# gvanhorn38/multibox

Hardware: AMD Instinct MI355X
Metric: images/sec (299x299, 5-AR priors) train (higher is better)
Workload: dtype bf16; 1 GPU; full train step: Inception-ResNet-v2 + multibox heads fwd, on-device matching+loss, bwd, RMSProp+EMA; 299x299, k=5 (P=646), BATCH_SIZE=64/GPU, MAX_NUM_BBOXES=13; global_batch=64, parallelism=dp1, hip_graph=True

## Files before the change

### include/mbx.h

```cpp
#ifndef MBX_H
#define MBX_H

#include <stddef.h>
#include <stdint.h>

#ifdef __cplusplus
extern "C" {
#endif

typedef void* mbx_stream_t;

typedef enum {
  MBX_OK = 0,
  MBX_ERR_INVALID_ARG = -1,
  MBX_ERR_UNSUPPORTED = -2,
  MBX_ERR_LAUNCH = -3,
  MBX_ERR_WORKSPACE = -4
} mbx_status;

int mbx_version(void);
const char* mbx_status_string(int status);

int mbx_priors_count(int k, const int* grids, int n_grids);

// ... 13 lines not shown
              void* workspace, size_t workspace_bytes, mbx_stream_t stream);

int mbx_match_extend(const float* priors , const float* gt ,
                     const int32_t* n_gt , const int32_t* status ,
                     float iou_threshold, int B, int P, int G,
                     int32_t* match ,
                     int32_t* n_extra , mbx_stream_t stream);

int mbx_match_atss_supported(int P, int G, int n_levels, const int32_t* level_start , int topk);
int mbx_match_atss(const float* priors , const int32_t* level_start ,
                   int n_levels, const float* gt , const int32_t* n_gt ,
                   const int32_t* status , int topk, int B, int P, int G,
                   int32_t* match , int32_t* n_extra ,
                   double* thr , mbx_stream_t stream);

size_t mbx_loss_workspace_bytes(int B);
int mbx_loss_fwd_bwd(const float* decoded , const float* conf_in ,
                     int conf_is_logit, const float* gt ,
                     const int32_t* match , float alpha, float grad_scale, int B, int P,
                     int G, float* loss2 ,
                     float* d_raw_locs , float* d_logits ,
                     void* workspace, size_t workspace_bytes, mbx_stream_t stream);

size_t mbx_loss_mined_workspace_bytes(int B, int P);
int mbx_loss_fwd_bwd_mined(const float* decoded , const float* conf_in ,
                           int conf_is_logit, const float* gt ,
                           const int32_t* match , float alpha, float grad_scale, int B, int P,
                           int G, float* loss2 ,
                           float* d_raw_locs , float* d_logits ,
                           int neg_per_pos, int min_neg, int32_t* n_neg ,
                           void* workspace, size_t workspace_bytes, mbx_stream_t stream);

size_t mbx_loss_focal_workspace_bytes(int B, int P);
int mbx_loss_fwd_bwd_focal(const float* decoded , const float* conf_in ,
                           int conf_is_logit, const float* gt ,
                           const int32_t* match , float alpha, float grad_scale, int B, int P,
                           int G, float* loss2 ,
                           float* d_raw_locs , float* d_logits ,
                           float gamma, float w_pos, float w_neg,
                           int neg_per_pos , int min_neg, int32_t* n_neg ,
                           void* workspace, size_t workspace_bytes, mbx_stream_t stream);

enum { MBX_LOC_L2 = 0, MBX_LOC_SMOOTH_L1 = 1, MBX_LOC_GIOU = 2, MBX_LOC_DIOU = 3, MBX_LOC_CIOU = 4 };
size_t mbx_loss_loc_workspace_bytes(int B, int P);
int mbx_loss_fwd_bwd_loc(const float* decoded , const float* conf_in ,
                         int conf_is_logit, const float* gt ,
                         const int32_t* match , float alpha, float grad_scale, int B, int P,
                         int G, float* loss2 ,
                         float* d_raw_locs , float* d_logits ,
                         int loc_type , float loc_beta ,
                         float gamma, float w_pos, float w_neg,
                         int neg_per_pos , int min_neg, int32_t* n_neg ,
                         void* workspace, size_t workspace_bytes, mbx_stream_t stream);

typedef struct {
  int32_t offset_y, offset_x;
  int32_t patch_h, patch_w;
  int32_t image_h, image_w;
  int32_t is_flipped;
  int32_t max_to_keep;
  float restrictions[4];
} mbx_patch_meta;

int mbx_decode_filter_topk(const float* raw_locs , const float* conf ,
                           const float* priors , const mbx_patch_meta* meta ,
                           int B, int P, int k_max, double* out_boxes ,
                           float* out_scores , int32_t* out_index ,
                           int32_t* out_count , mbx_stream_t stream);

int mbx_nms(double* boxes , float* scores , int32_t* index ,
            int32_t* count , int B, int k_max, double iou_threshold, mbx_stream_t stream);

#define MBX_MERGE_MAX_CANDIDATES 16384
int mbx_merge_detections(const double* boxes , const float* scores ,
                         const int32_t* count , const int32_t* image_rows , int I, int k_max,
                         int max_det, double iou_threshold, double* out_boxes ,
                         float* out_scores , int32_t* out_src ,
                         int32_t* out_count , int32_t* out_status , mbx_stream_t stream);

int mbx_merge_detections_voted(const double* boxes , const float* scores ,
                               const int32_t* count , const int32_t* image_rows , int I,
                               int k_max, int max_det, double iou_threshold, double vote_iou_threshold,
                               double* out_boxes , float* out_scores ,
                               int32_t* out_src , int32_t* out_count ,
                               int32_t* out_status , int32_t* out_votes , mbx_stream_t stream);

#define MBX_SOFT_LINEAR 1
#define MBX_SOFT_GAUSSIAN 2
int mbx_merge_detections_soft(const double* boxes , const float* scores ,
                              const int32_t* count , const int32_t* image_rows , int I, int k_max,
                              int max_det, int method, double iou_threshold , double sigma ,
                              double min_score, double vote_iou_threshold ,
                              double* out_boxes , float* out_scores ,
                              int32_t* out_src , int32_t* out_count , int32_t* out_status ,
                              int32_t* out_votes , mbx_stream_t stream);

#define MBX_COCO_MAX_DET 100
#define MBX_COCO_MAX_GT 128
int mbx_coco_match(const double* dt , const int32_t* dt_rows ,
                   const double* gt , const int32_t* gt_rows , int I,
                   const double* iou_thrs , int T, const double* area_rng ,
                   int A, int16_t* match , uint8_t* ignore ,
                   int32_t* n_gt_counted , int32_t* status , mbx_stream_t stream);

#define MBX_COCO_ACC_MAX_R 128
#define MBX_COCO_ACC_MAX_M 4
// ... 146 lines not shown
int mbx_bn_bwd_reduce(const void* da, int ld_da, const void* a, int ld_a, int relu, const void* y,
                      int64_t M, int C, const float* mean, const float* rstd, const float* beta,
                      float* partial , mbx_stream_t stream);
int mbx_bn_bwd_finalize(const float* partial, int rows, int C, int64_t M, float* dbeta ,
                        float* m12 , mbx_stream_t stream);
int mbx_bn_bwd_apply(const void* da, int ld_da, const void* a, int ld_a, int relu, const void* y,
                     int64_t M, int C, const float* mean, const float* rstd, const float* beta,
                     const float* m12, void* dy , mbx_stream_t stream);

int mbx_bn_bwd_reduce_mapped(const void* da, int ld_da, const void* a, int ld_a, int relu, const void* y, int64_t M, int C,
                             const float* mean, const float* rstd, const float* beta, float* partial,
                             const mbx_chan_map* da_map , mbx_stream_t stream);
int mbx_bn_bwd_apply_mapped(const void* da, int ld_da, const void* a, int ld_a, int relu, const void* y, int64_t M, int C,
                            const float* mean, const float* rstd, const float* beta, const float* m12, void* dy,
                            const mbx_chan_map* da_map , mbx_stream_t stream);

int mbx_bn_bwd_apply_rows(const float* stats, int rows, const void* da, int ld_da, const void* y, int64_t M, int C,
                          const float* mean, const float* rstd, const float* relu_thr, float* dbeta, void* dy,
                          const mbx_chan_map* da_map , mbx_stream_t stream);

size_t mbx_bn_bwd_onepass_workspace_bytes(int C);
int mbx_bn_bwd_onepass_supported(int64_t M, int C, int max_workgroups);
int mbx_bn_bwd_onepass(const void* da, int ld_da, int relu, const void* y, int64_t M, int C,
                       const float* mean, const float* rstd, const float* beta, float* dbeta ,
                       void* dy , void* ws, int max_workgroups, float* step_poison ,
                       mbx_stream_t stream);

int mbx_bn_bwd_rows_pooled(int N, int H, int W, int C);
int mbx_bn_bwd_reduce_pooled(const void* gy, int64_t gy_img_stride, int ld_gy, const uint8_t* argmax, int N, int H, int W,
                             int Ho, int Wo, int relu, const void* y, int C, const float* mean, const float* rstd,
                             const float* beta, float* partial , mbx_stream_t stream);
int mbx_bn_bwd_apply_pooled(const void* gy, int64_t gy_img_stride, int ld_gy, const uint8_t* argmax, int N, int H, int W,
                            int Ho, int Wo, int relu, const void* y, int C, const float* mean, const float* rstd,
                            const float* beta, const float* m12, void* dy, mbx_stream_t stream);
int mbx_bn_bwd_onepass_mapped(const void* da, int ld_da, int relu, const void* y, int64_t M, int C, const float* mean,
                              const float* rstd, const float* beta, float* dbeta, void* dy, void* ws, int max_workgroups,
                              float* step_poison, const mbx_chan_map* da_map , mbx_stream_t stream);

int mbx_maxpool_fwd(const void* x, int64_t x_img_stride, int ldx, int N, int H, int W, int C,
                    int k, int stride, void* y, int64_t y_img_stride, int ldy, int Ho, int Wo,
                    uint8_t* argmax , mbx_stream_t stream);
int mbx_maxpool_bwd(const void* dy, int64_t dy_img_stride, int ld_dy, const uint8_t* argmax,
                    int N, int H, int W, int C, int k, int stride, int Ho, int Wo, void* dx,
                    int64_t dx_img_stride, int ld_dx, int accumulate, mbx_stream_t stream);
int mbx_avgpool_fwd(const void* x, int64_t x_img_stride, int ldx, int N, int H, int W, int C,
                    int k, int pad, void* y, int64_t y_img_stride, int ldy, int Ho, int Wo,
                    mbx_stream_t stream);
int mbx_avgpool_bwd(const void* dy, int64_t dy_img_stride, int ld_dy, int N, int H, int W, int C,
                    int k, int pad, int Ho, int Wo, void* dx, int64_t dx_img_stride, int ld_dx,
                    int accumulate, mbx_stream_t stream);

int mbx_relu_mask(void* g, int ld_g, const void* a, int ld_a, int64_t M, int C, mbx_stream_t stream);
int mbx_pack_input(const float* img, int64_t pixels, void* out, mbx_stream_t stream);
int mbx_head_gather(const float* h, int ld_h, int N, int cells, int k, int P, int off,
                    float* locs, float* logits, mbx_stream_t stream);
int mbx_head_scatter(const float* d_locs, const float* d_logits, int N, int cells, int k, int P,
                     int off, void* g, int ld_g, mbx_stream_t stream);

typedef struct {
  const float* h; int32_t ld_h;
  void* g; int32_t ld_g;
  int32_t cells, k, off;
} mbx_head;
int mbx_head_gather_all(const mbx_head* heads , int n_heads, int N, int P, float* locs, float* logits,
                        mbx_stream_t stream);
int mbx_head_scatter_all(const float* d_locs, const float* d_logits, const mbx_head* heads , int n_heads, int N,
                         int P, mbx_stream_t stream);

int mbx_step_begin(float* grads, int64_t n_grads, float* bn_ws, int64_t n_ws, int64_t ctl_index, uint64_t* timeouts_total,
                   float* zero_scalar, mbx_stream_t stream);

typedef struct {
  int64_t src_off;
  int64_t dst_off;
  int32_t K, R, S, C, Kpad;
  int32_t first_block;
} mbx_filter_entry;
int mbx_filter_prepare(const void* w_bf16, void* w_dgrad, const mbx_filter_entry* table ,
                       int n_entries, int total_blocks, mbx_stream_t stream);

int mbx_rmsprop_ema_step(float* w, const float* g, float* ms, float* mom ,
                         float* ema , void* w_bf16 , int64_t n, float lr,
                         float decay, float momentum, float eps, float wd, float ema_decay,
                         int trainable, float* reg_loss, const float* skip_ctl, mbx_stream_t stream);
int mbx_ema_update(float* ema, const float* value, int64_t n, float ema_decay, const float* skip_ctl ,
                   mbx_stream_t stream);

int64_t mbx_grad_sqnorm_partials(int64_t n);
int mbx_grad_sqnorm(const float* g, const float* w , int64_t n, float wd, double* partials,
                    mbx_stream_t stream);
int mbx_clip_finalize(const double* partials, int64_t n_slots, double max_norm, const float* ctl, float* clip ,
                      int64_t* counts , mbx_stream_t stream);
int mbx_rmsprop_ema_step_clipped(float* w, const float* g, float* ms, float* mom ,
                                 float* ema , void* w_bf16 , int64_t n, float lr,
                                 float decay, float momentum, float eps, float wd, float ema_decay,
                                 int trainable, float* reg_loss, const float* clip, mbx_stream_t stream);

int mbx_sgd_ema_step(float* w, const float* g, float* mom , float* ema ,
                     void* w_bf16 , int64_t n, float lr, float momentum, int nesterov, float wd_l2, float ema_decay,
                     int trainable, float* reg_loss, const float* ctl, int clipped, mbx_stream_t stream);
int mbx_adam_ema_step(float* w, const float* g, float* m, float* v, float* ema , void* w_bf16 ,
                      int64_t n, float lr, float beta1, float beta2, float eps, float wd_l2, float wd_decoupled, int64_t calls,
                      const int64_t* skipped , float ema_decay, int trainable, float* reg_loss,
                      const float* ctl, int clipped, mbx_stream_t stream);

typedef struct { int64_t lo; int32_t len; int32_t var; } mbx_trust_chunk;
typedef struct { int32_t first_chunk; int32_t n_chunks; int32_t adapt; int32_t pad; } mbx_trust_var;
int64_t mbx_trust_chunk_elems(void);
int64_t mbx_trust_plan_count(const int64_t* bounds , int64_t n_vars);
int mbx_trust_plan(const int64_t* bounds , const int32_t* adapt , int64_t n_vars,
                   mbx_trust_chunk* chunks_out , mbx_trust_var* vars_out );
int mbx_trust_norms_sgd(const float* w, const float* g, const mbx_trust_chunk* chunks, int64_t n_chunks, float wd_l2,
                        double* partials , const float* ctl, int clipped, mbx_stream_t stream);
int mbx_trust_moments_adam(const float* w, const float* g, float* m, float* v, const mbx_trust_chunk* chunks, int64_t n_chunks,
                           float beta1, float beta2, float eps, float wd_l2, float wd_decoupled, int64_t calls,
                           const int64_t* skipped , double* partials , const float* ctl,
                           int clipped, mbx_stream_t stream);
int mbx_trust_ratios(const double* partials, const mbx_trust_var* vars, int64_t n_vars, float coeff, float* ratio ,
                     const float* ctl, mbx_stream_t stream);
int mbx_sgd_ema_step_trust(float* w, const float* g, float* mom , float* ema ,
                           void* w_bf16 , int64_t n, float lr, float momentum, int nesterov, float wd_l2,
                           float ema_decay, int trainable, float* reg_loss, const float* ctl, int clipped,
                           const mbx_trust_chunk* chunks, int64_t n_chunks, const float* ratio, mbx_stream_t stream);
// ... 35 lines not shown
```

### multibox_amd/_lib.py

```python
from __future__ import annotations

import ctypes as C
import os

_HERE = os.path.dirname(os.path.abspath(__file__))
LIB_PATH = os.path.join(_HERE, "libmbx.so")

P = C.c_void_p
I = C.c_int
F = C.c_float
D = C.c_double
SZ = C.c_size_t


class PatchMeta(C.Structure):
    _fields_ = [("offset_y", C.c_int32), ("offset_x", C.c_int32), ("patch_h", C.c_int32), ("patch_w", C.c_int32),
                ("image_h", C.c_int32), ("image_w", C.c_int32), ("is_flipped", C.c_int32),
                ("max_to_keep", C.c_int32), ("restrictions", C.c_float * 4)]


_SIGS = {
    "mbx_version": (I, []),
    "mbx_status_string": (C.c_char_p, [I]),
    "mbx_priors_count": (I, [I, P, I]),
    "mbx_crc32c": (C.c_uint32, [P, C.c_uint64, C.c_uint32]),
    "mbx_generate_priors": (I, [P, I, D, D, I, P, I, P]),
    "mbx_decode_conf": (I, [P, P, P, I, I, F, P, P, P]),
    "mbx_match_workspace_bytes": (SZ, [I, I, I]),
    "mbx_match": (I, [P, P, P, P, F, I, I, I, P, P, P, SZ, P]),
    "mbx_match_extend": (I, [P, P, P, P, F, I, I, I, P, P, P]),
    "mbx_match_atss_supported": (I, [I, I, I, P, I]),
    "mbx_match_atss": (I, [P, P, I, P, P, P, I, I, I, I, P, P, P, P]),
    "mbx_loss_workspace_bytes": (SZ, [I]),
    "mbx_loss_fwd_bwd": (I, [P, P, I, P, P, F, F, I, I, I, P, P, P, P, SZ, P]),
    "mbx_loss_mined_workspace_bytes": (SZ, [I, I]),
    "mbx_loss_fwd_bwd_mined": (I, [P, P, I, P, P, F, F, I, I, I, P, P, P, I, I, P, P, SZ, P]),
    "mbx_loss_focal_workspace_bytes": (SZ, [I, I]),
    "mbx_loss_fwd_bwd_focal": (I, [P, P, I, P, P, F, F, I, I, I, P, P, P, F, F, F, I, I, P, P, SZ, P]),
    "mbx_loss_loc_workspace_bytes": (SZ, [I, I]),
    "mbx_loss_fwd_bwd_loc": (I, [P, P, I, P, P, F, F, I, I, I, P, P, P, I, F, F, F, F, I, I, P, P, SZ, P]),
    "mbx_decode_filter_topk": (I, [P, P, P, P, I, I, I, P, P, P, P, P]),
    "mbx_nms": (I, [P, P, P, P, I, I, C.c_double, P]),
    "mbx_merge_detections": (I, [P, P, P, P, I, I, I, C.c_double, P, P, P, P, P, P]),
    "mbx_merge_detections_voted": (I, [P, P, P, P, I, I, I, C.c_double, C.c_double, P, P, P, P, P, P, P]),
    "mbx_merge_detections_soft": (I, [P, P, P, P, I, I, I, I, C.c_double, C.c_double, C.c_double, C.c_double, P, P, P, P, P, P, P]),
    "mbx_coco_match": (I, [P, P, P, P, I, P, I, P, I, P, P, P, P, P]),
    "mbx_coco_accumulate_workspace": (SZ, [C.c_longlong, I, I, I]),
    "mbx_coco_accumulate": (I, [P, P, I, P, P, P, I, I, P, I, P, I, P, P, P, SZ, P]),
    "mbx_augment_workspace_bytes": (SZ, [I, I]),
    "mbx_augment_batch": (I, [P, P, I, I, I, P, P, P]),
    "mbx_extract_patches": (I, [P, P, I, I, P, P]),
    "mbx_conv_stats_rows": (I, [P]),
    "mbx_conv": (I, [P, P]),
    "mbx_conv_supported": (I, [P]),
    "mbx_conv_pair": (I, [P, P, P]),
    "mbx_conv_splitk_workspace_bytes": (SZ, [P]),
    "mbx_conv_wgrad": (I, [P, P, C.c_int64, I, P, P, P]),
    "mbx_conv_wgrad_scaled": (I, [P, P, C.c_int64, I, F, P, P, P]),
    "mbx_wgrad_plan_bytes": (SZ, [P, I, I]),
    "mbx_wgrad_plan": (I, [P, I, I, P, SZ, P]),
    "mbx_conv_wgrad_grouped": (I, [P, P, P]),
    "mbx_conv_wgrad_grouped_capped": (I, [P, P, I, P]),
    "mbx_bn_finalize": (I, [P, I, I, C.c_int64, F, F, P, P, P, P, P]),
    "mbx_bn_apply": (I, [P, C.c_int64, I, P, P, P, I, P, I, P]),
    "mbx_bn_moving_update": (I, [P, P, P, P, C.c_int64, F, P, P, P, P, F, P]),
    "mbx_bn_finalize_parts": (I, [P, P, P, I, C.c_int64, F, F, P, P, P, P, P]),
    "mbx_bn_apply_mapped": (I, [P, C.c_int64, I, P, P, P, I, P, I, P, P]),
    "mbx_bn_bwd_reduce_mapped": (I, [P, I, P, I, I, P, C.c_int64, I, P, P, P, P, P, P]),
    "mbx_bn_bwd_apply_mapped": (I, [P, I, P, I, I, P, C.c_int64, I, P, P, P, P, P, P, P]),
    "mbx_bn_apply_maxpool": (I, [P, I, I, I, I, P, P, P, I, P, C.c_int64, I, I, I, P, P]),
    "mbx_bn_bwd_rows_pooled": (I, [I, I, I, I]),
    "mbx_bn_bwd_reduce_pooled": (I, [P, C.c_int64, I, P, I, I, I, I, I, I, P, I, P, P, P, P, P]),
    "mbx_bn_bwd_apply_pooled": (I, [P, C.c_int64, I, P, I, I, I, I, I, I, P, I, P, P, P, P, P, P]),
    "mbx_bn_bwd_onepass_mapped": (I, [P, I, I, P, C.c_int64, I, P, P, P, P, P, P, I, P, P, P]),
    "mbx_bn_fold": (I, [P, P, P, F, I, P, P, P]),
    "mbx_bn_apply_fused": (I, [P, I, C.c_int64, F, F, P, C.c_int64, I, P, I, P, I, P, P, P, P, P]),
    "mbx_bn_apply_fused_mapped": (I, [P, I, C.c_int64, F, F, P, C.c_int64, I, P, I, P, I, P, P, P, P, P, P, P]),
    "mbx_bn_bwd_apply_rows": (I, [P, I, P, I, P, C.c_int64, I, P, P, P, P, P, P, P]),
    "mbx_bn_bwd_rows": (I, [C.c_int64, I]),
    "mbx_bn_bwd_onepass_workspace_bytes": (C.c_size_t, [I]),
    "mbx_bn_bwd_onepass_supported": (I, [C.c_int64, I, I]),
    "mbx_bn_bwd_onepass": (I, [P, I, I, P, C.c_int64, I, P, P, P, P, P, P, I, P, P]),
    "mbx_bn_bwd_reduce": (I, [P, I, P, I, I, P, C.c_int64, I, P, P, P, P, P]),
    "mbx_bn_bwd_finalize": (I, [P, I, I, C.c_int64, P, P, P]),
    "mbx_bn_bwd_apply": (I, [P, I, P, I, I, P, C.c_int64, I, P, P, P, P, P, P]),
    "mbx_maxpool_fwd": (I, [P, C.c_int64, I, I, I, I, I, I, I, P, C.c_int64, I, I, I, P, P]),
    "mbx_maxpool_bwd": (I, [P, C.c_int64, I, P, I, I, I, I, I, I, I, I, P, C.c_int64, I, I, P]),
    "mbx_avgpool_fwd": (I, [P, C.c_int64, I, I, I, I, I, I, I, P, C.c_int64, I, I, I, P]),
    "mbx_avgpool_bwd": (I, [P, C.c_int64, I, I, I, I, I, I, I, I, I, P, C.c_int64, I, I, P]),
    "mbx_relu_mask": (I, [P, I, P, I, C.c_int64, I, P]),
    "mbx_pack_input": (I, [P, C.c_int64, P, P]),
    "mbx_head_gather": (I, [P, I, I, I, I, I, I, P, P, P]),
    "mbx_head_scatter": (I, [P, P, I, I, I, I, I, P, I, P]),
    "mbx_head_gather_all": (I, [P, I, I, I, P, P, P]),
    "mbx_head_scatter_all": (I, [P, P, P, I, I, I, P]),
    "mbx_step_begin": (I, [P, C.c_int64, P, C.c_int64, C.c_int64, P, P, P]),
    "mbx_filter_prepare": (I, [P, P, P, I, I, P]),
    "mbx_rmsprop_ema_step": (I, [P, P, P, P, P, P, C.c_int64, F, F, F, F, F, F, I, P, P, P]),
    "mbx_ema_update": (I, [P, P, C.c_int64, F, P, P]),
    "mbx_grad_sqnorm_partials": (C.c_int64, [C.c_int64]),
    "mbx_grad_sqnorm": (I, [P, P, C.c_int64, F, P, P]),
    "mbx_clip_finalize": (I, [P, C.c_int64, D, P, P, P, P]),
    "mbx_rmsprop_ema_step_clipped": (I, [P, P, P, P, P, P, C.c_int64, F, F, F, F, F, F, I, P, P, P]),
    "mbx_sgd_ema_step": (I, [P, P, P, P, P, C.c_int64, F, F, I, F, F, I, P, P, I, P]),
    "mbx_adam_ema_step": (I, [P, P, P, P, P, P, C.c_int64, F, F, F, F, F, F, C.c_int64, P, F, I, P, P, I, P]),
    "mbx_trust_chunk_elems": (C.c_int64, []),
    "mbx_trust_plan_count": (C.c_int64, [P, C.c_int64]),
    "mbx_trust_plan": (I, [P, P, C.c_int64, P, P]),
    "mbx_trust_norms_sgd": (I, [P, P, P, C.c_int64, F, P, P, I, P]),
    "mbx_trust_moments_adam": (I, [P, P, P, P, P, C.c_int64, F, F, F, F, F, C.c_int64, P, P, P, I, P]),
    "mbx_trust_ratios": (I, [P, P, C.c_int64, F, P, P, P]),
    "mbx_sgd_ema_step_trust": (I, [P, P, P, P, P, C.c_int64, F, F, I, F, F, I, P, P, I, P, C.c_int64, P, P]),
    "mbx_adam_ema_step_trust": (I, [P, P, P, P, P, P, C.c_int64, F, F, F, F, F, F, C.c_int64, P, F, I, P, P, I, P, C.c_int64, P, P]),
}

_lib = None


class MbxError(RuntimeError):
    pass


class ChanMap(C.Structure):
    _fields_ = [("n", C.c_int32), ("c_begin", C.c_int32 * 4), ("offset", C.c_int32 * 4)]


class BnBwdStats(C.Structure):
    _fields_ = [("n", C.c_int32), ("rows_mod", C.c_int32), ("c_begin", C.c_int32 * 4), ("y", C.c_void_p * 4), ("ld_y", C.c_int32 * 4),
                ("relu_thr", C.c_void_p * 4), ("stats", C.c_void_p * 4), ("stats_ld", C.c_int32 * 4)]


class Head(C.Structure):
    _fields_ = [("h", C.c_void_p), ("ld_h", C.c_int32), ("g", C.c_void_p), ("ld_g", C.c_int32), ("cells", C.c_int32),
                ("k", C.c_int32), ("off", C.c_int32)]


class TrustChunk(C.Structure):
    _fields_ = [("lo", C.c_int64), ("len", C.c_int32), ("var", C.c_int32)]


class TrustVar(C.Structure):
    _fields_ = [("first_chunk", C.c_int32), ("n_chunks", C.c_int32), ("adapt", C.c_int32), ("pad", C.c_int32)]


# ... 30 lines not shown
```

### multibox_amd/csrc/loss.hip

```cpp
#include "boxes.h"

namespace {

constexpr int kThreads = 256;
constexpr int kWaves = kThreads / 64;

__global__ void __launch_bounds__(kThreads)
decode_conf_kernel(const float4* __restrict__ raw, const float* __restrict__ logits,
                   const float4* __restrict__ priors, int total, int P, float eps_add,
                   float4* __restrict__ decoded, float* __restrict__ conf) {
  for (int i = blockIdx.x * blockDim.x + threadIdx.x; i < total; i += gridDim.x * blockDim.x) {
    if (decoded) {
      const float4 r = raw[i], p = priors[i % P];
      decoded[i] = make_float4(__fadd_rn(r.x, p.x), __fadd_rn(r.y, p.y), __fadd_rn(r.z, p.z), __fadd_rn(r.w, p.w));
    }
    if (conf) {
      const float s = 1.0f / (1.0f + expf(-logits[i]));
      conf[i] = __fadd_rn(s, eps_add);
    }
  }
}

__device__ __forceinline__ double match_cost(const float4 l, const float4 g, float half_alpha,
                                             float lc, float l1c) {
  const float d0 = __fsub_rn(l.x, g.x), d1 = __fsub_rn(l.y, g.y), d2 = __fsub_rn(l.z, g.z), d3 = __fsub_rn(l.w, g.w);
  const float ss = __fadd_rn(__fadd_rn(__fadd_rn(__fmul_rn(d0, d0), __fmul_rn(d1, d1)), __fmul_rn(d2, d2)), __fmul_rn(d3, d3));
  const float nrm = __fsqrt_rn(ss);
  float t = __fmul_rn(half_alpha, __fmul_rn(nrm, nrm));
  t = __fsub_rn(t, lc);
  t = __fadd_rn(t, l1c);
  return (double)t;
}

struct Cand {
  double val;
  int j;
  int free_;
};

__device__ __forceinline__ bool cand_better(const Cand& a, const Cand& b) {
  if (a.j < 0) return false;
  if (b.j < 0) return true;
  if (a.val < b.val) return true;
  if (a.val > b.val) return false;
  if (a.free_ != b.free_) return a.free_ > b.free_;
  return a.j < b.j;
}

__device__ __forceinline__ Cand cand_shfl_xor(const Cand& c, int o) {
  Cand r;
  r.val = __shfl_xor(c.val, o, 64);
  r.j = __shfl_xor(c.j, o, 64);
  r.free_ = __shfl_xor(c.free_, o, 64);
  return r;
}

__global__ void __launch_bounds__(1024)
match_kernel(const float4* __restrict__ decoded, const float* __restrict__ conf,
             const float4* __restrict__ gt, const int* __restrict__ n_gt, float alpha, int P, int G,
             int* __restrict__ match, int* __restrict__ status) {
  extern __shared__ __attribute__((aligned(16))) unsigned char smem[];
  double* v = reinterpret_cast<double*>(smem);
  double* spc = v + P;
  double* u = spc + P;
  float2* lcl = reinterpret_cast<float2*>(u + G);
  int* path = reinterpret_cast<int*>(lcl + P);
  int* row4col = path + P;
  int* SC = row4col + P;
  int* col4row = SC + P;
  int* SR = col4row + G;
  __shared__ Cand wave_best[16];
  __shared__ int sh_i, sh_sink, sh_bad;
  __shared__ double sh_min;
// ... 58 lines not shown
        Cand c; c.val = s; c.j = j; c.free_ = row4col[j] < 0;
        if (cand_better(c, best)) best = c;
      }
#pragma unroll
      for (int o = 32; o > 0; o >>= 1) {
        const Cand other = cand_shfl_xor(best, o);
        if (cand_better(other, best)) best = other;
      }
      if ((tid & 63) == 0) wave_best[tid >> 6] = best;
      __syncthreads();
      if (tid == 0) {
        Cand bb = wave_best[0];
        for (int w = 1; w < nwaves; ++w) if (cand_better(wave_best[w], bb)) bb = wave_best[w];
        if (bb.j < 0 || !(bb.val < INFINITY)) {
          sh_sink = -2;
        } else {
          sh_min = bb.val;
          SC[bb.j] = 1;
          SR[i] = 1;
          const int r4c = row4col[bb.j];
          if (r4c < 0) sh_sink = bb.j; else sh_i = r4c;
        }
      }
      __syncthreads();
      if (sh_sink != -1) break;
    }
    const int sink = sh_sink;
    if (sink == -2) { if (tid == 0) status[b] = 2; return; }
    const double min_val = sh_min;
    for (int i = tid; i < n; i += nt) {
      if (i == cur) u[i] += min_val;
      else if (SR[i]) u[i] += min_val - spc[col4row[i]];
    }
    for (int j = tid; j < P; j += nt)
      if (SC[j]) v[j] -= min_val - spc[j];
    __syncthreads();
    if (tid == 0) {
      int j = sink;
      while (true) {
        const int i = path[j];
        row4col[j] = i;
        const int t = col4row[i];
        col4row[i] = j;
        j = t;
        if (i == cur) break;
      }
    }
    __syncthreads();
  }
  for (int i = tid; i < n; i += nt) mt[col4row[i]] = i;
  if (tid == 0) status[b] = 0;
}

struct StagedBox { Box box; double area; };

__global__ void __launch_bounds__(1024)
match_extend_kernel(const float4* __restrict__ priors, const float4* __restrict__ gt, const int* __restrict__ n_gt,
                    const int* __restrict__ status, double thr, int P, int G, int* __restrict__ match,
                    int* __restrict__ n_extra) {
  extern __shared__ __attribute__((aligned(16))) unsigned char smem[];
  StagedBox* boxes = reinterpret_cast<StagedBox*>(smem);
  __shared__ int added_waves[16];
  const int b = blockIdx.x, tid = threadIdx.x, nt = (int)blockDim.x;
  const int n = n_gt[b];
  if (status[b] != 0 || n <= 0 || n > G) {
    if (tid == 0 && n_extra) n_extra[b] = 0;
    return;
  }
  for (int j = tid; j < n; j += nt) {
    const float4 q = gt[(size_t)b * G + j];
    StagedBox s;
    s.box = {(double)q.x, (double)q.y, (double)q.z, (double)q.w};
    s.area = box_area(s.box);
    boxes[j] = s;
  }
  __syncthreads();
  int* mt = match + (size_t)b * P;
  int added = 0;
  for (int p = tid; p < P; p += nt) {
    if (mt[p] >= 0) continue;
    const float4 q = priors[p];
    const Box e = {(double)q.x, (double)q.y, (double)q.z, (double)q.w};
    const double area_e = box_area(e);
    double best = thr;
    int best_j = -1;
    for (int j = 0; j < n; ++j) {
      const Box g = boxes[j].box;
      const double iw = fmin(e.x2, g.x2) - fmax(e.x1, g.x1), ih = fmin(e.y2, g.y2) - fmax(e.y1, g.y1);
      if (iw > 0.0 && ih > 0.0) {
        const double inter = iw * ih;
        const double uni = area_e + boxes[j].area - inter;
        const double iou = uni > 0.0 ? inter / uni : 0.0;
        if (iou > best) { best = iou; best_j = j; }
      }
    }
    if (best_j >= 0) { mt[p] = best_j; ++added; }
  }
  if (!n_extra) return;
  added = wave_sum(added);
  if ((tid & 63) == 0) added_waves[tid >> 6] = added;
  __syncthreads();
  if (tid == 0) {
    int total = 0;
    for (int w = 0; w < (nt >> 6); ++w) total += added_waves[w];
    n_extra[b] = total;
  }
}

struct AtssLevels { int start[9]; };

__device__ __forceinline__ void wave_lds_sync() {
  __builtin_amdgcn_fence(__ATOMIC_RELEASE, "wavefront");
  __builtin_amdgcn_wave_barrier();
  __builtin_amdgcn_fence(__ATOMIC_ACQUIRE, "wavefront");
}

__device__ __forceinline__ unsigned long long atss_d2_key(const float4 q, double cxj, double cyj) {
  const double cx = ((double)q.x + (double)q.z) * 0.5, cy = ((double)q.y + (double)q.w) * 0.5;
  const double dx = cx - cxj, dy = cy - cyj;
  const double d2 = dx * dx + dy * dy;
  return d2 != d2 ? ~0ull : (d2 == 0.0 ? 0ull : (unsigned long long)__double_as_longlong(d2));
}

__device__ __forceinline__ bool atss_pair_less(unsigned long long ka, int ia, unsigned long long kb, int ib) {
  return ka < kb || (ka == kb && ia < ib);
}

template <int CTRL, int ROW_MASK>
__device__ __forceinline__ void atss_dpp_min(unsigned long long& k) {
  const unsigned olo = (unsigned)__builtin_amdgcn_update_dpp(-1, (int)(unsigned)k, CTRL, ROW_MASK, 0xf, false);
  const unsigned ohi = (unsigned)__builtin_amdgcn_update_dpp(-1, (int)(unsigned)(k >> 32), CTRL, ROW_MASK, 0xf, false);
  const unsigned long long ok = ((unsigned long long)ohi << 32) | olo;
  if (ok < k) k = ok;
}
template <int CTRL, int ROW_MASK>
__device__ __forceinline__ void atss_dpp_min(int& i) {
  const int oi = __builtin_amdgcn_update_dpp(0x7fffffff, i, CTRL, ROW_MASK, 0xf, false);
  if (oi < i) i = oi;
}
template <typename T>
__device__ __forceinline__ void atss_dpp_min_to_lane63(T& v) {
  atss_dpp_min<0x111, 0xf>(v);
  atss_dpp_min<0x112, 0xf>(v);
  atss_dpp_min<0x114, 0xf>(v);
  atss_dpp_min<0x118, 0xf>(v);
  atss_dpp_min<0x142, 0xa>(v);
  atss_dpp_min<0x143, 0xc>(v);
}

__device__ __forceinline__ void atss_wave_min(unsigned long long& k, int& i) {
  unsigned long long mk = k;
  atss_dpp_min_to_lane63(mk);
  const unsigned lo = (unsigned)__builtin_amdgcn_readlane((int)(unsigned)mk, 63);
  const unsigned hi = (unsigned)__builtin_amdgcn_readlane((int)(unsigned)(mk >> 32), 63);
  mk = ((unsigned long long)hi << 32) | lo;
  const unsigned long long tied = __ballot(k == mk);
  int mi;
  if (__popcll(tied) == 1) {
    mi = __builtin_amdgcn_readlane(i, __ffsll((long long)tied) - 1);
  } else {
    mi = k == mk ? i : 0x7fffffff;
    atss_dpp_min_to_lane63(mi);
    mi = __builtin_amdgcn_readlane(mi, 63);
  }
  k = mk;
  i = mi;
}

constexpr unsigned short kAtssNone = 0xffffu;
constexpr int kAtssKeep = 4;

__global__ void __launch_bounds__(1024)
match_atss_kernel(const float4* __restrict__ priors, const AtssLevels lv, int n_levels, const float4* __restrict__ gt,
                  const int* __restrict__ n_gt, const int* __restrict__ status, int topk, int m, int P, int G,
                  int* __restrict__ match, int* __restrict__ n_extra, double* __restrict__ thr_out) {
  extern __shared__ __attribute__((aligned(16))) unsigned char smem[];
  const int b = blockIdx.x, tid = threadIdx.x, nt = (int)blockDim.x, lane = tid & 63, wave = tid >> 6, nw = nt >> 6;
  unsigned long long* claim = reinterpret_cast<unsigned long long*>(smem);
  StagedBox* boxes = reinterpret_cast<StagedBox*>(claim + P);
  double* iou_w = reinterpret_cast<double*>(boxes + G) + (size_t)wave * m;
  unsigned short* cand = reinterpret_cast<unsigned short*>(reinterpret_cast<double*>(boxes + G) + (size_t)nw * m);
  __shared__ int ls[9];
  __shared__ int added_waves[16];
  const int n = n_gt[b];
  if (status[b] != 0 || n <= 0 || n > G) {
    if (tid == 0 && n_extra) n_extra[b] = 0;
    if (thr_out) for (int j = tid; j < G; j += nt) thr_out[(size_t)b * G + j] = 0.0;
    return;
  }
  if (tid == 0) {
#pragma unroll
    for (int i = 0; i < 9; ++i) ls[i] = lv.start[i];
  }
  for (int p = tid; p < P; p += nt) claim[p] = 0ull;
  for (int j = tid; j < n; j += nt) {
    const float4 q = gt[(size_t)b * G + j];
    StagedBox s;
    s.box = {(double)q.x, (double)q.y, (double)q.z, (double)q.w};
    s.area = box_area(s.box);
    boxes[j] = s;
// ... 247 lines not shown
      if (mt[p] >= 0) continue;
      const unsigned long long key = mined_key(cf[p], P, p);
      if (((key ^ cut) & fixed) == 0ull) atomicAdd(&hist[(unsigned)(key >> shift) & 255u], 1u);
    }
    __syncthreads();
    if (tid < 64) {
      const unsigned h0 = hist[4 * tid], h1 = hist[4 * tid + 1], h2 = hist[4 * tid + 2], h3 = hist[4 * tid + 3];
      const unsigned own = h0 + h1 + h2 + h3;
      unsigned incl = own;
#pragma unroll
      for (int o = 1; o < 64; o <<= 1) {
        const unsigned t = __shfl_down(incl, o, 64);
        if (tid + o < 64) incl += t;
      }
      bool whole = false;
      if (shift == 56) {
        const int n_negatives = (int)__shfl(incl, 0, 64), n_pos = P - n_negatives;
        long long K = (long long)neg_per_pos * (long long)n_pos;
        if (K < (long long)min_neg) K = min_neg;
        if (K > (long long)n_negatives) K = n_negatives;
        need = (int)K;
        whole = need == 0 || need == n_negatives;
        if (tid == 0) {
          if (n_neg) n_neg[b] = need;
          if (whole) { sh_cut = need == 0 ? ~0ull : 0ull; sh_need = 0; sh_done = 1; }
        }
      }
      const unsigned above = incl - own, k = (unsigned)need;
      if (!whole && above < k && k <= incl) {
        unsigned a = above, cnt = h3;
        int d = 3;
        if (k > a + h3) { a += h3; cnt = h2; d = 2;
          if (k > a + h2) { a += h2; cnt = h1; d = 1;
            if (k > a + h1) { a += h1; cnt = h0; d = 0; } } }
        sh_cut = cut | ((unsigned long long)(4 * tid + d) << shift);
        sh_need = (int)(k - a);
        sh_done = cnt == k - a;
      }
    }
    __syncthreads();
    cut = sh_cut;
    need = sh_need;
    if (sh_done) break;
  }
  return cut;
}

template <bool MINED, bool FOCAL, bool LOC_ANY>
__device__ __forceinline__ void loss_body(const float4* __restrict__ decoded, const float* __restrict__ logits, int is_logit,
                                          const float4* __restrict__ gt, const int* __restrict__ match, float alpha,
                                          float grad_scale, int P, int G, int loc_type, float loc_beta, float gamma,
                                          float w_pos, float w_neg, int neg_per_pos, int min_neg,
                                          double* __restrict__ partial , float4* __restrict__ d_locs,
                                          float* __restrict__ d_logits, int* __restrict__ n_neg) {
  constexpr bool kCountPositives = FOCAL && !MINED;
  const int b = blockIdx.x, tid = threadIdx.x;
  unsigned long long cut = 0ull;
  if (MINED) cut = mined_select_cut(match + (size_t)b * P, logits + (size_t)b * P, P, neg_per_pos, min_neg, b, n_neg);
  const bool modulated = FOCAL && gamma != 0.0f;

  double loc_acc = 0.0, conf_acc = 0.0;
  int n_pos = 0;
  for (int p = tid; p < P; p += kThreads) {
    const size_t i = (size_t)b * P + p;
    const int m = match[i];
    const float z = logits[i];
    float4 dl = make_float4(0.f, 0.f, 0.f, 0.f);
    float g;
    if (MINED && m < 0 && mined_key(z, P, p) < cut) {
      g = 0.f;
    } else {
      const float s = is_logit ? 1.0f / (1.0f + expf(-z)) : z;
      const float c = __fadd_rn(s, 1e-10f);
      const float w = __fadd_rn(__fsub_rn(1.0f, c), 1e-10f);
      const float ds = is_logit ? s * (1.0f - s) : 1.0f;
      const bool pos = m >= 0;
      if (pos) {
        const float4 l = decoded[i], q = gt[(size_t)b * G + m];
        if (!LOC_ANY || loc_type == MBX_LOC_L2) {
          const float d0 = __fsub_rn(l.x, q.x), d1 = __fsub_rn(l.y, q.y), d2 = __fsub_rn(l.z, q.z), d3 = __fsub_rn(l.w, q.w);
          loc_acc += (double)d0 * d0 + (double)d1 * d1 + (double)d2 * d2 + (double)d3 * d3;
          const float a = alpha * grad_scale;
          dl = make_float4(a * d0, a * d1, a * d2, a * d3);
        } else {
          double dx1, dy1, dx2, dy2;
          loc_acc += loc_term(loc_type, (double)loc_beta, l, q, dx1, dy1, dx2, dy2);
          const double a = (double)alpha * (double)grad_scale;
          dl = make_float4((float)(a * dx1), (float)(a * dy1), (float)(a * dx2), (float)(a * dy2));
        }
        if (kCountPositives) ++n_pos;
      }
      const float arg = pos ? c : w, base = pos ? w : c, wt = FOCAL ? (pos ? w_pos : w_neg) : 1.0f;
      const float lg = logf(arg);
      const float pw = modulated ? powf(base, gamma) : 1.0f;
      conf_acc -= (double)wt * ((double)pw * (double)lg);
      float d = (ds * pw) / arg;
      if (modulated) d = d - gamma * (pw / base) * lg * ds;
      d = wt * d;
      g = (pos ? -d : d) * grad_scale;
    }
    if (d_locs) d_locs[i] = dl;
    if (d_logits) d_logits[i] = g;
  }
  loc_acc = wave_sum(loc_acc);
  conf_acc = wave_sum(conf_acc);
  __shared__ double red[kWaves][2];
  __shared__ int pos_waves[kWaves];
  if (kCountPositives) n_pos = wave_sum(n_pos);
  if ((tid & 63) == 0) {
    red[tid >> 6][0] = loc_acc; red[tid >> 6][1] = conf_acc;
    if (kCountPositives) pos_waves[tid >> 6] = n_pos;
  }
  __syncthreads();
  if (tid == 0) {
    double a = 0.0, c = 0.0;
    for (int w = 0; w < kWaves; ++w) { a += red[w][0]; c += red[w][1]; }
    partial[2 * b] = a;
    partial[2 * b + 1] = c;
    if (kCountPositives && n_neg) {
      int total = 0;
      for (int w = 0; w < kWaves; ++w) total += pos_waves[w];
      n_neg[b] = P - total;
    }
  }
}

__global__ void __launch_bounds__(kThreads)
loss_kernel(const float4* __restrict__ decoded, const float* __restrict__ logits, int is_logit,
            const float4* __restrict__ gt, const int* __restrict__ match, float alpha, float grad_scale,
            int P, int G, double* __restrict__ partial , float4* __restrict__ d_locs,
            float* __restrict__ d_logits) {
  loss_body<false, false, false>(decoded, logits, is_logit, gt, match, alpha, grad_scale, P, G, MBX_LOC_L2, 0.0f, 0.0f, 1.0f,
                                 1.0f, 0, 0, partial, d_locs, d_logits, nullptr);
}

__global__ void __launch_bounds__(kThreads)
loss_mined_kernel(const float4* __restrict__ decoded, const float* __restrict__ logits, int is_logit,
                  const float4* __restrict__ gt, const int* __restrict__ match, float alpha, float grad_scale,
                  int P, int G, int neg_per_pos, int min_neg, double* __restrict__ partial ,
                  float4* __restrict__ d_locs, float* __restrict__ d_logits, int* __restrict__ n_neg) {
  loss_body<true, false, false>(decoded, logits, is_logit, gt, match, alpha, grad_scale, P, G, MBX_LOC_L2, 0.0f, 0.0f, 1.0f,
                                1.0f, neg_per_pos, min_neg, partial, d_locs, d_logits, n_neg);
}

template <bool MINED>
__global__ void __launch_bounds__(kThreads)
loss_focal_kernel(const float4* __restrict__ decoded, const float* __restrict__ logits, int is_logit,
                  const float4* __restrict__ gt, const int* __restrict__ match, float alpha, float grad_scale,
                  int P, int G, float gamma, float w_pos, float w_neg, int neg_per_pos, int min_neg,
                  double* __restrict__ partial , float4* __restrict__ d_locs, float* __restrict__ d_logits,
                  int* __restrict__ n_neg) {
  loss_body<MINED, true, false>(decoded, logits, is_logit, gt, match, alpha, grad_scale, P, G, MBX_LOC_L2, 0.0f, gamma, w_pos,
                                w_neg, neg_per_pos, min_neg, partial, d_locs, d_logits, n_neg);
}

template <bool MINED>
__global__ void __launch_bounds__(kThreads)
loss_loc_kernel(const float4* __restrict__ decoded, const float* __restrict__ logits, int is_logit,
                const float4* __restrict__ gt, const int* __restrict__ match, float alpha, float grad_scale,
                int P, int G, int loc_type, float loc_beta, float gamma, float w_pos, float w_neg, int neg_per_pos,
                int min_neg, double* __restrict__ partial , float4* __restrict__ d_locs,
                float* __restrict__ d_logits, int* __restrict__ n_neg) {
  loss_body<MINED, true, true>(decoded, logits, is_logit, gt, match, alpha, grad_scale, P, G, loc_type, loc_beta, gamma, w_pos,
                               w_neg, neg_per_pos, min_neg, partial, d_locs, d_logits, n_neg);
}

}

extern "C" int mbx_decode_conf(const float* raw_locs, const float* logits, const float* priors, int B,
                               int P, float eps_add, float* decoded, float* conf, mbx_stream_t stream) {
  if (B < 0 || P <= 0) return MBX_ERR_INVALID_ARG;
  if ((decoded && (!raw_locs || !priors)) || (conf && !logits)) return MBX_ERR_INVALID_ARG;
  if (B == 0 || (!decoded && !conf)) return MBX_OK;
  const int total = B * P;
  int blocks = (total + kThreads - 1) / kThreads;
  if (blocks > 2048) blocks = 2048;
  MBX_ENTER();
  hipLaunchKernelGGL(decode_conf_kernel, dim3(blocks), dim3(kThreads), 0, mbx_s(stream),
                     reinterpret_cast<const float4*>(raw_locs), logits, reinterpret_cast<const float4*>(priors),
                     total, P, eps_add, reinterpret_cast<float4*>(decoded), conf);
  MBX_LAUNCH_CHECK();
  return MBX_OK;
}

static size_t match_lds_bytes(int P, int G) { return (size_t)P * 36 + (size_t)G * 16 + 16; }

extern "C" size_t mbx_match_workspace_bytes(int, int, int) { return 0; }

extern "C" int mbx_match(const float* decoded, const float* conf, const float* gt, const int32_t* n_gt,
                         float alpha, int B, int P, int G, int32_t* match, int32_t* status, void*, size_t,
                         mbx_stream_t stream) {
  if (!decoded || !conf || !gt || !n_gt || !match || !status || B < 0 || P <= 0 || G <= 0) return MBX_ERR_INVALID_ARG;
  if (B == 0) return MBX_OK;
  const size_t lds = match_lds_bytes(P, G);
  if (lds > 150 * 1024) return MBX_ERR_UNSUPPORTED;
  static const int force_nt = mbx_env_int("MBX_MATCH_THREADS", 0);
  const int nthreads = force_nt ? force_nt : (P > 1536 ? 512 : kThreads);
  MBX_ENTER();
  if (lds > 64 * 1024) {
    if (hipFuncSetAttribute(reinterpret_cast<const void*>(match_kernel), hipFuncAttributeMaxDynamicSharedMemorySize,
                            (int)lds) != hipSuccess) return MBX_ERR_LAUNCH;
  }
  hipLaunchKernelGGL(match_kernel, dim3(B), dim3(nthreads), lds, mbx_s(stream),
                     reinterpret_cast<const float4*>(decoded), conf, reinterpret_cast<const float4*>(gt), n_gt,
                     alpha, P, G, match, status);
  MBX_LAUNCH_CHECK();
  return MBX_OK;
}

extern "C" int mbx_match_extend(const float* priors, const float* gt, const int32_t* n_gt, const int32_t* status,
                                float iou_threshold, int B, int P, int G, int32_t* match, int32_t* n_extra,
                                mbx_stream_t stream) {
  if (!priors || !gt || !n_gt || !status || !match || B < 0 || P <= 0 || G <= 0) return MBX_ERR_INVALID_ARG;
  if (!(iou_threshold > 0.0f && iou_threshold <= 1.0f)) return MBX_ERR_INVALID_ARG;
  const size_t lds = (size_t)G * sizeof(StagedBox);
  if (lds > 60 * 1024) return MBX_ERR_UNSUPPORTED;
  if (B == 0) return MBX_OK;
  const int nthreads = P >= 1024 ? 1024 : (P + 63) / 64 * 64;
  MBX_ENTER();
  hipLaunchKernelGGL(match_extend_kernel, dim3(B), dim3(nthreads), lds, mbx_s(stream),
                     reinterpret_cast<const float4*>(priors), reinterpret_cast<const float4*>(gt), n_gt, status,
                     (double)iou_threshold, P, G, match, n_extra);
  MBX_LAUNCH_CHECK();
  return MBX_OK;
}

static int atss_plan(int P, int G, int n_levels, const int32_t* level_start, int topk, int* m_out, int* waves_out,
                     size_t* lds_out) {
  if (!level_start || P <= 0 || G <= 0 || topk < 1 || n_levels < 1 || n_levels > 8) return MBX_ERR_INVALID_ARG;
  if (level_start[0] != 0 || level_start[n_levels] != P) return MBX_ERR_INVALID_ARG;
  long long m = 0;
  for (int l = 0; l < n_levels; ++l) {
    const int size = level_start[l + 1] - level_start[l];
    if (level_start[l + 1] <= level_start[l]) return MBX_ERR_INVALID_ARG;
    m += topk < size ? topk : size;
  }
  if (P >= (int)kAtssNone) return MBX_ERR_UNSUPPORTED;
  for (int waves = 16; waves >= 1; waves >>= 1) {
    const long long lds = 8ll * P + (long long)sizeof(StagedBox) * G + 2ll * G * m + 8ll * waves * m;
    if (lds + 128 <= 64 * 1024) {
      if (m_out) *m_out = (int)m;
      if (waves_out) *waves_out = waves;
      if (lds_out) *lds_out = (size_t)lds;
      return MBX_OK;
    }
  }
  return MBX_ERR_UNSUPPORTED;
}

extern "C" int mbx_match_atss_supported(int P, int G, int n_levels, const int32_t* level_start, int topk) {
  return atss_plan(P, G, n_levels, level_start, topk, nullptr, nullptr, nullptr);
}

extern "C" int mbx_match_atss(const float* priors, const int32_t* level_start, int n_levels, const float* gt,
                              const int32_t* n_gt, const int32_t* status, int topk, int B, int P, int G, int32_t* match,
                              int32_t* n_extra, double* thr, mbx_stream_t stream) {
  if (!priors || !gt || !n_gt || !status || !match || B < 0) return MBX_ERR_INVALID_ARG;
  int m = 0, waves = 0;
  size_t lds = 0;
  const int plan = atss_plan(P, G, n_levels, level_start, topk, &m, &waves, &lds);
  if (plan != MBX_OK) return plan;
  if (B == 0) return MBX_OK;
  AtssLevels lv;
  for (int i = 0; i < 9; ++i) lv.start[i] = i <= n_levels ? level_start[i] : P;
  MBX_ENTER();
  hipLaunchKernelGGL(match_atss_kernel, dim3(B), dim3(waves * 64), lds, mbx_s(stream),
                     reinterpret_cast<const float4*>(priors), lv, n_levels, reinterpret_cast<const float4*>(gt), n_gt,
                     status, topk, m, P, G, match, n_extra, thr);
  MBX_LAUNCH_CHECK();
  return MBX_OK;
}

extern "C" size_t mbx_loss_workspace_bytes(int B) { return (size_t)(B > 0 ? B : 1) * 2 * sizeof(double); }
extern "C" size_t mbx_loss_mined_workspace_bytes(int B, int) { return mbx_loss_workspace_bytes(B); }
extern "C" size_t mbx_loss_focal_workspace_bytes(int B, int) { return mbx_loss_workspace_bytes(B); }
extern "C" size_t mbx_loss_loc_workspace_bytes(int B, int) { return mbx_loss_workspace_bytes(B); }

enum class LossKind { kPlain, kMined, kFocal, kLoc };

static int launch_loss(LossKind kind, const float* decoded, const float* logits, int conf_is_logit, const float* gt,
                       const int32_t* match, float alpha, float grad_scale, int B, int P, int G, float* loss2,
                       float* d_raw_locs, float* d_logits, int loc_type, float loc_beta, float gamma, float w_pos,
                       float w_neg, int neg_per_pos, int min_neg, int32_t* n_neg, void* workspace, size_t workspace_bytes,
                       mbx_stream_t stream) {
  if (!decoded || !logits || !gt || !match || !loss2 || B <= 0 || P <= 0 || G <= 0) return MBX_ERR_INVALID_ARG;
  if (!workspace || workspace_bytes < mbx_loss_workspace_bytes(B)) return MBX_ERR_WORKSPACE;
  double* partial = reinterpret_cast<double*>(workspace);
  const float4* dec4 = reinterpret_cast<const float4*>(decoded);
  const float4* gt4 = reinterpret_cast<const float4*>(gt);
  float4* dl4 = reinterpret_cast<float4*>(d_raw_locs);
  MBX_ENTER();
  switch (kind) {
    case LossKind::kPlain:
      hipLaunchKernelGGL(loss_kernel, dim3(B), dim3(kThreads), 0, mbx_s(stream), dec4, logits, conf_is_logit, gt4, match,
                         alpha, grad_scale, P, G, partial, dl4, d_logits);
      break;
    case LossKind::kMined:
      hipLaunchKernelGGL(loss_mined_kernel, dim3(B), dim3(kThreads), 0, mbx_s(stream), dec4, logits, conf_is_logit, gt4,
                         match, alpha, grad_scale, P, G, neg_per_pos, min_neg, partial, dl4, d_logits, n_neg);
      break;
    case LossKind::kFocal:
      hipLaunchKernelGGL(neg_per_pos ? loss_focal_kernel<true> : loss_focal_kernel<false>, dim3(B), dim3(kThreads), 0,
                         mbx_s(stream), dec4, logits, conf_is_logit, gt4, match, alpha, grad_scale, P, G, gamma, w_pos,
                         w_neg, neg_per_pos, min_neg, partial, dl4, d_logits, n_neg);
      break;
    case LossKind::kLoc:
      hipLaunchKernelGGL(neg_per_pos ? loss_loc_kernel<true> : loss_loc_kernel<false>, dim3(B), dim3(kThreads), 0,
                         mbx_s(stream), dec4, logits, conf_is_logit, gt4, match, alpha, grad_scale, P, G, loc_type, loc_beta,
                         gamma, w_pos, w_neg, neg_per_pos, min_neg, partial, dl4, d_logits, n_neg);
      break;
  }
  MBX_LAUNCH_CHECK();
  hipLaunchKernelGGL(loss_final_kernel, dim3(1), dim3(64), 0, mbx_s(stream), partial, B, alpha,
                     loc_type == MBX_LOC_L2 ? 0.5 : 1.0, loss2);
  MBX_LAUNCH_CHECK();
  return MBX_OK;
}

extern "C" int mbx_loss_fwd_bwd(const float* decoded, const float* logits, int conf_is_logit, const float* gt,
                                const int32_t* match, float alpha, float grad_scale, int B, int P, int G, float* loss2,
                                float* d_raw_locs, float* d_logits, void* workspace, size_t workspace_bytes,
                                mbx_stream_t stream) {
  return launch_loss(LossKind::kPlain, decoded, logits, conf_is_logit, gt, match, alpha, grad_scale, B, P, G, loss2,
                     d_raw_locs, d_logits, MBX_LOC_L2, 0.0f, 0.0f, 1.0f, 1.0f, 0, 0, nullptr, workspace, workspace_bytes, stream);
}

extern "C" int mbx_loss_fwd_bwd_mined(const float* decoded, const float* logits, int conf_is_logit, const float* gt,
                                      const int32_t* match, float alpha, float grad_scale, int B, int P, int G, float* loss2,
                                      float* d_raw_locs, float* d_logits, int neg_per_pos, int min_neg, int32_t* n_neg,
                                      void* workspace, size_t workspace_bytes, mbx_stream_t stream) {
  if (neg_per_pos < 1 || min_neg < 0) return MBX_ERR_INVALID_ARG;
  return launch_loss(LossKind::kMined, decoded, logits, conf_is_logit, gt, match, alpha, grad_scale, B, P, G, loss2,
                     d_raw_locs, d_logits, MBX_LOC_L2, 0.0f, 0.0f, 1.0f, 1.0f, neg_per_pos, min_neg, n_neg, workspace,
                     workspace_bytes, stream);
}

static bool focal_arguments_ok(float gamma, float w_pos, float w_neg, int neg_per_pos, int min_neg) {
  if (!(gamma >= 0.0f && gamma <= 10.0f)) return false;
  if (!(w_pos >= 0.0f && w_neg >= 0.0f) || isinf(w_pos) || isinf(w_neg)) return false;
  return !(neg_per_pos < 0 || min_neg < 0 || (neg_per_pos == 0 && min_neg > 0));
}

extern "C" int mbx_loss_fwd_bwd_focal(const float* decoded, const float* logits, int conf_is_logit, const float* gt,
                                      const int32_t* match, float alpha, float grad_scale, int B, int P, int G, float* loss2,
                                      float* d_raw_locs, float* d_logits, float gamma, float w_pos, float w_neg,
                                      int neg_per_pos, int min_neg, int32_t* n_neg, void* workspace, size_t workspace_bytes,
                                      mbx_stream_t stream) {
  if (!focal_arguments_ok(gamma, w_pos, w_neg, neg_per_pos, min_neg)) return MBX_ERR_INVALID_ARG;
  return launch_loss(LossKind::kFocal, decoded, logits, conf_is_logit, gt, match, alpha, grad_scale, B, P, G, loss2,
                     d_raw_locs, d_logits, MBX_LOC_L2, 0.0f, gamma, w_pos, w_neg, neg_per_pos, min_neg, n_neg, workspace,
                     workspace_bytes, stream);
}

extern "C" int mbx_loss_fwd_bwd_loc(const float* decoded, const float* logits, int conf_is_logit, const float* gt,
                                    const int32_t* match, float alpha, float grad_scale, int B, int P, int G, float* loss2,
                                    float* d_raw_locs, float* d_logits, int loc_type, float loc_beta, float gamma, float w_pos,
                                    float w_neg, int neg_per_pos, int min_neg, int32_t* n_neg, void* workspace,
                                    size_t workspace_bytes, mbx_stream_t stream) {
  if (loc_type < MBX_LOC_L2 || loc_type > MBX_LOC_CIOU) return MBX_ERR_INVALID_ARG;
  if (loc_type == MBX_LOC_SMOOTH_L1 && !(loc_beta > 0.0f && !isinf(loc_beta))) return MBX_ERR_INVALID_ARG;
  if (!focal_arguments_ok(gamma, w_pos, w_neg, neg_per_pos, min_neg)) return MBX_ERR_INVALID_ARG;
  return launch_loss(LossKind::kLoc, decoded, logits, conf_is_logit, gt, match, alpha, grad_scale, B, P, G, loss2,
                     d_raw_locs, d_logits, loc_type, loc_beta, gamma, w_pos, w_neg, neg_per_pos, min_neg, n_neg, workspace,
                     workspace_bytes, stream);
}
```

### multibox_amd/csrc/nnops.hip

```cpp
#include "optim_rules.h"
#include <type_traits>

namespace {

template <int KK, int SS>
__global__ void __launch_bounds__(kT)
maxpool_fwd_kernel(const unsigned short* __restrict__ x, long long xs, int ldx, int N, int H, int W, int C, int k_,
                   int stride_, unsigned short* __restrict__ y, long long ys, int ldy, int Ho, int Wo,
                   unsigned char* __restrict__ argmax) {
  const int k = KK ? KK : k_, stride = SS ? SS : stride_;
  const int C8 = C >> 3;
  const unsigned total = (unsigned)N * Ho * Wo * C8;
  for (unsigned i = blockIdx.x * kT + threadIdx.x; i < total; i += gridDim.x * kT) {
    unsigned t = i / (unsigned)C8;
    const int c = (int)(i - t * C8) << 3;
    const unsigned t2 = t / (unsigned)Wo;
    const int ow = (int)(t - t2 * Wo);
    const int n = (int)(t2 / (unsigned)Ho);
    const int oh = (int)(t2 - (unsigned)n * Ho);
    float best[8];
    unsigned arg[8];
#pragma unroll
    for (int j = 0; j < 8; ++j) { best[j] = -INFINITY; arg[j] = 0; }
    if constexpr (KK > 0) {
// ... 213 lines not shown
#pragma unroll
      for (int a = 0; a < 3; ++a)
#pragma unroll
        for (int b = 0; b < 3; ++b) {
          const int oh = oh0 + a, ow = ow0 + b;
          const bool ok = oh <= oh1 && ow <= ow1;
          const int nh = min(oh - pad + 3, H) - max(oh - pad, 0), nw = min(ow - pad + 3, W) - max(ow - pad, 0);
          inv[a * 3 + b] = ok ? 1.0f / (float)(nh * nw) : 0.f;
          v[a * 3 + b] = ok ? ld8(dy + n * dys + ((long long)oh * Wo + ow) * ld_dy + c) : u32x4{0u, 0u, 0u, 0u};
        }
#pragma unroll
      for (int tq = 0; tq < 9; ++tq) {
        if (inv[tq] == 0.f) continue;
        float g[8];
        unpack8(v[tq], g);
#pragma unroll
        for (int j = 0; j < 8; ++j) acc[j] += g[j] * inv[tq];
      }
    } else
    for (int oh = oh0; oh <= oh1; ++oh) {
      const int nh = min(oh - pad + k, H) - max(oh - pad, 0);
      for (int ow = ow0; ow <= ow1; ++ow) {
        const int nw = min(ow - pad + k, W) - max(ow - pad, 0);
        const float inv = 1.0f / (float)(nh * nw);
        float g[8];
        unpack8(ld8(dy + n * dys + ((long long)oh * Wo + ow) * ld_dy + c), g);
#pragma unroll
        for (int j = 0; j < 8; ++j) acc[j] += g[j] * inv;
      }
    }
    st8(dst, pack8(acc));
  }
}

__global__ void __launch_bounds__(kT)
relu_mask_kernel(unsigned short* __restrict__ g, int ld_g, const unsigned short* __restrict__ a, int ld_a,
                 long long M, int C) {
  const int C8 = C >> 3;
  const long long total = M * C8;
  for (long long i = (long long)blockIdx.x * kT + threadIdx.x; i < total; i += (long long)gridDim.x * kT) {
    const long long m = i / C8;
    const int c = (int)(i - m * C8) << 3;
    float gg[8], aa[8];
    unpack8(ld8(g + m * ld_g + c), gg);
    unpack8(ld8(a + m * ld_a + c), aa);
#pragma unroll
    for (int j = 0; j < 8; ++j)
      if (!(aa[j] > 0.f)) gg[j] = 0.f;
    st8(g + m * ld_g + c, pack8(gg));
  }
}

__global__ void __launch_bounds__(kT)
pack_input_kernel(const float* __restrict__ img, long long pixels, unsigned short* __restrict__ out) {
  for (long long i = (long long)blockIdx.x * kT + threadIdx.x; i < pixels; i += (long long)gridDim.x * kT) {
    float f[8] = {img[3 * i], img[3 * i + 1], img[3 * i + 2], 0.f, 0.f, 0.f, 0.f, 0.f};
    st8(out + 8 * i, pack8(f));
  }
}

__global__ void __launch_bounds__(kT)
head_gather_kernel(const float* __restrict__ h, int ld_h, int N, int cells, int k, int P, int off,
                   float* __restrict__ locs, float* __restrict__ logits) {
  const int total = N * cells * k;
  for (int i = blockIdx.x * kT + threadIdx.x; i < total; i += gridDim.x * kT) {
    const int a = i % k, t = i / k, cell = t % cells, n = t / cells;
    const float* row = h + (size_t)(n * cells + cell) * ld_h;
    const size_t p = (size_t)n * P + off + cell * k + a;
    *reinterpret_cast<float4*>(locs + p * 4) = make_float4(row[a * 4], row[a * 4 + 1], row[a * 4 + 2], row[a * 4 + 3]);
    logits[p] = row[4 * k + a];
  }
}

__global__ void __launch_bounds__(kT)
head_scatter_kernel(const float* __restrict__ d_locs, const float* __restrict__ d_logits, int N, int cells, int k,
                    int P, int off, unsigned short* __restrict__ g, int ld_g) {
  const int total = N * cells * ld_g;
  for (int i = blockIdx.x * kT + threadIdx.x; i < total; i += gridDim.x * kT) {
    const int ch = i % ld_g, t = i / ld_g, cell = t % cells, n = t / cells;
    const size_t p = (size_t)n * P + off + cell * k;
    float v = 0.f;
    if (ch < 4 * k) v = d_locs[(p + ch / 4) * 4 + (ch & 3)];
    else if (ch < 5 * k) v = d_logits[p + (ch - 4 * k)];
    g[i] = (unsigned short)f2bf(v);
  }
}

constexpr int kMaxHeads = 8;
struct HeadTable {
  const float* h[kMaxHeads]; unsigned short* g[kMaxHeads];
  int ld_h[kMaxHeads], ld_g[kMaxHeads], cells[kMaxHeads], k[kMaxHeads], off[kMaxHeads];
  int start[kMaxHeads + 1];
  int n;
};

__global__ void __launch_bounds__(kT)
head_gather_all_kernel(const HeadTable t, int P, float* __restrict__ locs, float* __restrict__ logits) {
  const int total = t.start[t.n];
  for (int i = blockIdx.x * kT + threadIdx.x; i < total; i += gridDim.x * kT) {
    int j = 0;
    while (j + 1 < t.n && i >= t.start[j + 1]) ++j;
    const int e = i - t.start[j], k = t.k[j], cells = t.cells[j];
    const int a = e % k, q = e / k, cell = q % cells, n = q / cells;
    const float* row = t.h[j] + (size_t)(n * cells + cell) * t.ld_h[j];
    const size_t p = (size_t)n * P + t.off[j] + cell * k + a;
    *reinterpret_cast<float4*>(locs + p * 4) = make_float4(row[a * 4], row[a * 4 + 1], row[a * 4 + 2], row[a * 4 + 3]);
    logits[p] = row[4 * k + a];
  }
}

__global__ void __launch_bounds__(kT)
head_scatter_all_kernel(const HeadTable t, int P, const float* __restrict__ d_locs, const float* __restrict__ d_logits) {
  const int total = t.start[t.n];
  for (int i = blockIdx.x * kT + threadIdx.x; i < total; i += gridDim.x * kT) {
    int j = 0;
    while (j + 1 < t.n && i >= t.start[j + 1]) ++j;
    const int e = i - t.start[j], k = t.k[j], cells = t.cells[j], ld = t.ld_g[j];
    const int ch = e % ld, q = e / ld, cell = q % cells, n = q / cells;
    const size_t p = (size_t)n * P + t.off[j] + cell * k;
    float v = 0.f;
    if (ch < 4 * k) v = d_locs[(p + ch / 4) * 4 + (ch & 3)];
    else if (ch < 5 * k) v = d_logits[p + (ch - 4 * k)];
    t.g[j][e] = (unsigned short)f2bf(v);
  }
}

__global__ void __launch_bounds__(kT)
step_begin_kernel(float* __restrict__ G, long long nG, float* __restrict__ ws, long long nws, long long ctl,
                  unsigned long long* __restrict__ timeouts_total, float* __restrict__ scalar) {
  if (scalar && blockIdx.x == 0 && threadIdx.x == 0) *scalar = 0.f;
  const long long n4 = nG >> 2, w4 = nws >> 2;
  const float4 z = make_float4(0.f, 0.f, 0.f, 0.f);
  for (long long i = (long long)blockIdx.x * kT + threadIdx.x; i < n4 + w4; i += (long long)gridDim.x * kT) {
    if (i < n4) {
      if (timeouts_total && i == (ctl >> 2)) {
        const float t = G[ctl];
        if (t > 0.f) *timeouts_total += (unsigned long long)t;
      }
      reinterpret_cast<float4*>(G)[i] = z;
    } else {
      reinterpret_cast<float4*>(ws)[i - n4] = z;
    }
  }
}

__global__ void __launch_bounds__(kT)
filter_prepare_kernel(const unsigned short* __restrict__ w, unsigned short* __restrict__ wd,
                      const mbx_filter_entry* __restrict__ table, int n_entries) {
  __shared__ __attribute__((aligned(16))) unsigned short tile[64][40];
  int lo = 0, hi = n_entries - 1;
  while (lo < hi) {
    const int mid = (lo + hi + 1) >> 1;
    if (table[mid].first_block <= (int)blockIdx.x) lo = mid; else hi = mid - 1;
  }
  const mbx_filter_entry e = table[lo];
  const int kt = (e.Kpad + 63) / 64, ct = (e.C + 31) / 32;
  int b = blockIdx.x - e.first_block;
  const int ck = b % kt; b /= kt;
  const int cc = b % ct; b /= ct;
  const int s = b % e.S, r = b / e.S;
  const unsigned short* src = w + e.src_off;
  unsigned short* dst = wd + e.dst_off;
  const int k0 = ck * 64, c0 = cc * 32;
  const long long tap_src = ((long long)(e.R - 1 - r) * e.S + (e.S - 1 - s)) * e.C;
  if (((e.C | e.Kpad) & 7) == 0 && ((e.src_off | e.dst_off) & 7) == 0) {
    static_assert(kT == 256, "one 16-byte chunk per thread");
    {
      const int kk = threadIdx.x >> 2, c = (threadIdx.x & 3) << 3;
      uint4 v = make_uint4(0u, 0u, 0u, 0u);
      if (k0 + kk < e.K && c0 + c < e.C)
        v = *reinterpret_cast<const uint4*>(src + (long long)(k0 + kk) * e.R * e.S * e.C + tap_src + c0 + c);
      *reinterpret_cast<uint4*>(&tile[kk][c]) = v;
    }
    __syncthreads();
    {
      const int c = threadIdx.x >> 3, kk = (threadIdx.x & 7) << 3;
      if (k0 + kk < e.Kpad && c0 + c < e.C) {
        unsigned q[4];
#pragma unroll
        for (int j = 0; j < 4; ++j) q[j] = (unsigned)tile[kk + 2 * j][c] | ((unsigned)tile[kk + 2 * j + 1][c] << 16);
        *reinterpret_cast<uint4*>(dst + (((long long)(c0 + c) * e.R + r) * e.S + s) * e.Kpad + k0 + kk) =
            make_uint4(q[0], q[1], q[2], q[3]);
      }
    }
    return;
  }
  for (int i = threadIdx.x; i < 64 * 32; i += kT) {
    const int kk = i >> 5, c = i & 31;
    unsigned short v = 0;
    if (k0 + kk < e.K && c0 + c < e.C) v = src[(long long)(k0 + kk) * e.R * e.S * e.C + tap_src + c0 + c];
    tile[kk][c] = v;
  }
  __syncthreads();
  for (int i = threadIdx.x; i < 64 * 32; i += kT) {
// ... 250 lines not shown
  return MBX_OK;
}

extern "C" int mbx_maxpool_bwd(const void* dy, int64_t dys, int ld_dy, const uint8_t* argmax, int N, int H, int W, int C,
                               int k, int stride, int Ho, int Wo, void* dx, int64_t dxs, int ld_dx, int accumulate,
                               mbx_stream_t stream) {
  if (!pool_args_ok(dy, ld_dy, dx, ld_dx, N, H, W, C, k, Ho, Wo) || !argmax || stride < 1) return MBX_ERR_INVALID_ARG;
  MBX_ENTER();
  if (k == 3 && stride == 2)
    hipLaunchKernelGGL((maxpool_bwd_kernel<3, 2>), dim3(grid_for((long long)N * H * W * (C / 8))), dim3(kT), 0, mbx_s(stream),
                       (cus)dy, (long long)dys, ld_dy, argmax, N, H, W, C, k, stride, Ho, Wo, (us)dx, (long long)dxs, ld_dx,
                       accumulate);
  else
    hipLaunchKernelGGL((maxpool_bwd_kernel<0, 0>), dim3(grid_for((long long)N * H * W * (C / 8))), dim3(kT), 0, mbx_s(stream),
                       (cus)dy, (long long)dys, ld_dy, argmax, N, H, W, C, k, stride, Ho, Wo, (us)dx, (long long)dxs, ld_dx,
                       accumulate);
  MBX_LAUNCH_CHECK();
  return MBX_OK;
}

extern "C" int mbx_avgpool_fwd(const void* x, int64_t xs, int ldx, int N, int H, int W, int C, int k, int pad, void* y,
                               int64_t ys, int ldy, int Ho, int Wo, mbx_stream_t stream) {
  if (!pool_args_ok(x, ldx, y, ldy, N, H, W, C, k, Ho, Wo) || pad < 0 || pad >= k) return MBX_ERR_INVALID_ARG;
  if (Ho != H + 2 * pad - k + 1 || Wo != W + 2 * pad - k + 1) return MBX_ERR_INVALID_ARG;
  MBX_ENTER();
  hipLaunchKernelGGL(avgpool_fwd_kernel, dim3(grid_for((long long)N * Ho * Wo * (C / 8))), dim3(kT), 0, mbx_s(stream),
                     (cus)x, (long long)xs, ldx, N, H, W, C, k, pad, (us)y, (long long)ys, ldy, Ho, Wo);
  MBX_LAUNCH_CHECK();
  return MBX_OK;
}

extern "C" int mbx_avgpool_bwd(const void* dy, int64_t dys, int ld_dy, int N, int H, int W, int C, int k, int pad, int Ho,
                               int Wo, void* dx, int64_t dxs, int ld_dx, int accumulate, mbx_stream_t stream) {
  if (!pool_args_ok(dy, ld_dy, dx, ld_dx, N, H, W, C, k, Ho, Wo) || pad < 0 || pad >= k) return MBX_ERR_INVALID_ARG;
  MBX_ENTER();
  hipLaunchKernelGGL(avgpool_bwd_kernel, dim3(grid_for((long long)N * H * W * (C / 8))), dim3(kT), 0, mbx_s(stream),
                     (cus)dy, (long long)dys, ld_dy, N, H, W, C, k, pad, Ho, Wo, (us)dx, (long long)dxs, ld_dx, accumulate);
  MBX_LAUNCH_CHECK();
  return MBX_OK;
}

extern "C" int mbx_relu_mask(void* g, int ld_g, const void* a, int ld_a, int64_t M, int C, mbx_stream_t stream) {
  if (!g || !a || M <= 0 || C <= 0 || C % 8 || ld_g % 8 || ld_a % 8 || !al16(g) || !al16(a)) return MBX_ERR_INVALID_ARG;
  MBX_ENTER();
  hipLaunchKernelGGL(relu_mask_kernel, dim3(grid_for(M * (C / 8))), dim3(kT), 0, mbx_s(stream), (us)g, ld_g, (cus)a, ld_a,
                     (long long)M, C);
  MBX_LAUNCH_CHECK();
  return MBX_OK;
}

extern "C" int mbx_pack_input(const float* img, int64_t pixels, void* out, mbx_stream_t stream) {
  if (!img || !out || pixels <= 0 || !al16(out)) return MBX_ERR_INVALID_ARG;
  MBX_ENTER();
  hipLaunchKernelGGL(pack_input_kernel, dim3(grid_for(pixels)), dim3(kT), 0, mbx_s(stream), img, (long long)pixels, (us)out);
  MBX_LAUNCH_CHECK();
  return MBX_OK;
}

extern "C" int mbx_head_gather(const float* h, int ld_h, int N, int cells, int k, int P, int off, float* locs,
                               float* logits, mbx_stream_t stream) {
  if (!h || !locs || !logits || N <= 0 || cells <= 0 || k <= 0 || ld_h < 5 * k || off < 0 || off + cells * k > P)
    return MBX_ERR_INVALID_ARG;
  MBX_ENTER();
  hipLaunchKernelGGL(head_gather_kernel, dim3(grid_for((long long)N * cells * k)), dim3(kT), 0, mbx_s(stream), h, ld_h, N,
                     cells, k, P, off, locs, logits);
  MBX_LAUNCH_CHECK();
  return MBX_OK;
}

extern "C" int mbx_head_scatter(const float* d_locs, const float* d_logits, int N, int cells, int k, int P, int off, void* g,
                                int ld_g, mbx_stream_t stream) {
  if (!d_locs || !d_logits || !g || N <= 0 || cells <= 0 || k <= 0 || ld_g < 5 * k || off < 0 || off + cells * k > P)
    return MBX_ERR_INVALID_ARG;
  MBX_ENTER();
  hipLaunchKernelGGL(head_scatter_kernel, dim3(grid_for((long long)N * cells * ld_g)), dim3(kT), 0, mbx_s(stream), d_locs,
                     d_logits, N, cells, k, P, off, (us)g, ld_g);
  MBX_LAUNCH_CHECK();
  return MBX_OK;
}

static int fill_head_table(const mbx_head* heads, int n_heads, int N, int P, bool scatter, HeadTable& t) {
  if (!heads || n_heads <= 0 || n_heads > kMaxHeads || N <= 0 || P <= 0) return MBX_ERR_INVALID_ARG;
  long long acc = 0;
  t.n = n_heads;
  for (int j = 0; j < n_heads; ++j) {
    const mbx_head& H = heads[j];
    if (H.cells <= 0 || H.k <= 0 || H.off < 0 || H.off + H.cells * H.k > P) return MBX_ERR_INVALID_ARG;
    if (scatter ? (!H.g || H.ld_g < 5 * H.k) : (!H.h || H.ld_h < 5 * H.k)) return MBX_ERR_INVALID_ARG;
    t.h[j] = H.h; t.g[j] = reinterpret_cast<unsigned short*>(H.g);
    t.ld_h[j] = H.ld_h; t.ld_g[j] = H.ld_g; t.cells[j] = H.cells; t.k[j] = H.k; t.off[j] = H.off;
    t.start[j] = (int)acc;
    acc += (long long)N * H.cells * (scatter ? H.ld_g : H.k);
    if (acc >= (1LL << 31)) return MBX_ERR_UNSUPPORTED;
  }
  for (int j = n_heads; j <= kMaxHeads; ++j) t.start[j] = (int)acc;
  return MBX_OK;
}

extern "C" int mbx_head_gather_all(const mbx_head* heads, int n_heads, int N, int P, float* locs, float* logits,
                                   mbx_stream_t stream) {
  if (!locs || !logits) return MBX_ERR_INVALID_ARG;
  HeadTable t;
  const int st = fill_head_table(heads, n_heads, N, P, false, t);
  if (st != MBX_OK) return st;
  MBX_ENTER();
  hipLaunchKernelGGL(head_gather_all_kernel, dim3(grid_for(t.start[t.n])), dim3(kT), 0, mbx_s(stream), t, P, locs, logits);
  MBX_LAUNCH_CHECK();
  return MBX_OK;
}

extern "C" int mbx_head_scatter_all(const float* d_locs, const float* d_logits, const mbx_head* heads, int n_heads, int N,
                                    int P, mbx_stream_t stream) {
  if (!d_locs || !d_logits) return MBX_ERR_INVALID_ARG;
  HeadTable t;
  const int st = fill_head_table(heads, n_heads, N, P, true, t);
  if (st != MBX_OK) return st;
  MBX_ENTER();
  hipLaunchKernelGGL(head_scatter_all_kernel, dim3(grid_for(t.start[t.n])), dim3(kT), 0, mbx_s(stream), t, P, d_locs, d_logits);
  MBX_LAUNCH_CHECK();
  return MBX_OK;
}

extern "C" int mbx_step_begin(float* grads, int64_t n_grads, float* bn_ws, int64_t n_ws, int64_t ctl_index,
                              uint64_t* timeouts_total, float* zero_scalar, mbx_stream_t stream) {
  if (!grads || n_grads <= 0 || n_grads % 4 || n_ws < 0 || n_ws % 4 || (n_ws && !bn_ws) || !al16(grads) || (bn_ws && !al16(bn_ws)) ||
      (timeouts_total && (ctl_index < 0 || ctl_index >= n_grads)))
    return MBX_ERR_INVALID_ARG;
  MBX_ENTER();
  hipLaunchKernelGGL(step_begin_kernel, dim3(grid_for((n_grads + n_ws) / 4)), dim3(kT), 0, mbx_s(stream), grads,
                     (long long)n_grads, bn_ws, (long long)n_ws, (long long)ctl_index,
                     reinterpret_cast<unsigned long long*>(timeouts_total), zero_scalar);
  MBX_LAUNCH_CHECK();
  return MBX_OK;
}

extern "C" int mbx_filter_prepare(const void* w_bf16, void* w_dgrad, const mbx_filter_entry* table, int n_entries,
                                  int total_blocks, mbx_stream_t stream) {
  if (!w_bf16 || !w_dgrad || !table || n_entries <= 0 || total_blocks <= 0) return MBX_ERR_INVALID_ARG;
  MBX_ENTER();
  hipLaunchKernelGGL(filter_prepare_kernel, dim3(total_blocks), dim3(kT), 0, mbx_s(stream), (cus)w_bf16, (us)w_dgrad, table,
                     n_entries);
  MBX_LAUNCH_CHECK();
  return MBX_OK;
}

extern "C" int mbx_rmsprop_ema_step(float* w, const float* g, float* ms, float* mom, float* ema, void* w_bf16, int64_t n,
                                    float lr, float decay, float momentum, float eps, float wd, float ema_decay,
                                    int trainable, float* reg_loss, const float* skip_ctl, mbx_stream_t stream) {
  if (!w || n <= 0 || (trainable && (!g || !ms))) return MBX_ERR_INVALID_ARG;
  if (trainable && momentum != 0.f && !mom) return MBX_ERR_INVALID_ARG;
  MBX_ENTER();
  hipLaunchKernelGGL(rmsprop_ema_kernel<false>, dim3(grid_for(n)), dim3(kT), 0, mbx_s(stream), w, g, ms, momentum != 0.f ? mom : nullptr,
                     ema, (us)w_bf16, (long long)n, lr, decay, momentum, eps, wd, ema_decay, trainable, reg_loss, skip_ctl);
  MBX_LAUNCH_CHECK();
  return MBX_OK;
}

extern "C" int mbx_rmsprop_ema_step_clipped(float* w, const float* g, float* ms, float* mom, float* ema, void* w_bf16, int64_t n,
                                            float lr, float decay, float momentum, float eps, float wd, float ema_decay,
                                            int trainable, float* reg_loss, const float* clip, mbx_stream_t stream) {
  if (!w || n <= 0 || (trainable && (!g || !ms)) || !clip) return MBX_ERR_INVALID_ARG;
  if (trainable && momentum != 0.f && !mom) return MBX_ERR_INVALID_ARG;
  MBX_ENTER();
  hipLaunchKernelGGL(rmsprop_ema_kernel<true>, dim3(grid_for(n)), dim3(kT), 0, mbx_s(stream), w, g, ms, momentum != 0.f ? mom : nullptr,
                     ema, (us)w_bf16, (long long)n, lr, decay, momentum, eps, wd, ema_decay, trainable, reg_loss, clip);
  MBX_LAUNCH_CHECK();
  return MBX_OK;
}

extern "C" int64_t mbx_grad_sqnorm_partials(int64_t n) { return n > 0 ? sqnorm_grid(n) : 0; }

extern "C" int mbx_grad_sqnorm(const float* g, const float* w, int64_t n, float wd, double* partials, mbx_stream_t stream) {
  if (!g || n <= 0 || !partials || (reinterpret_cast<uintptr_t>(partials) & 7) || !(wd == wd) || (wd != 0.f && !w))
    return MBX_ERR_INVALID_ARG;
  MBX_ENTER();
  if (wd != 0.f)
    hipLaunchKernelGGL(grad_sqnorm_kernel<true>, dim3(sqnorm_grid(n)), dim3(kT), 0, mbx_s(stream), g, w, (long long)n, wd, partials);
  else
    hipLaunchKernelGGL(grad_sqnorm_kernel<false>, dim3(sqnorm_grid(n)), dim3(kT), 0, mbx_s(stream), g, (const float*)nullptr,
                       (long long)n, 0.f, partials);
  MBX_LAUNCH_CHECK();
  return MBX_OK;
}

// ... 46 lines not shown
```

### multibox_amd/engine.py

```python
from __future__ import annotations

import ctypes as C
import math
import os
import re

import numpy as np
import torch

from . import _lib, ops
from .ops import View

BN_EPS = 0.001
STATS_ROWS = int(os.environ.get("MBX_STATS_ROWS", "8"))
WEIGHT_DECAY = 0.00004


def _same_pad(n, k, s):
    out = -(-n // s)
    total = max((out - 1) * s + k - n, 0)
    return out, total // 2


def _valid(n, k, s):
# ... 87 lines not shown
              o.skip.ch_off < hi and o.skip.ch_off + o.skip.C > lo]
        return r

    def segments(X):
        segs, c, end = [], X.x.ch_off, X.x.ch_off + X.x.C
        while c < end:
            m = member_at(X.x.buf, c)
            if m is None:
                return None
            n = min(end, m.out.ch_off + m.K) - c
            segs.append((c - X.x.ch_off, m, c - m.out.ch_off, n))
            c += n
        if len(segs) > 4 or any(sg[0] % align for sg in segs):
            return None
        return segs

    eligible = set(id(u) for u in units)
    while True:
        conv_ok = {}
        for X in fwd:
            if id(X) not in is_conv or not X.need_dx or not X.trainable or X.stride != 1:
                continue
            segs = segments(X)
            if segs is None or any(id(sg[1].unit) not in eligible for sg in segs):
                continue
            if len(readers(X.x.buf, X.x.ch_off, X.x.ch_off + X.x.C)) != 1:
                continue
            if consumer_ok(X):
                conv_ok[id(X)] = (X, segs)
        drop = set()
        for u in units:
            if id(u) not in eligible:
                continue
            for m in u.members:
                rd = readers(m.out.buf, m.out.ch_off, m.out.ch_off + m.K)
                covered = sorted((max(o.x.ch_off, m.out.ch_off), min(o.x.ch_off + o.x.C, m.out.ch_off + m.K)) for o in rd)
                tiled = bool(covered) and covered[0][0] == m.out.ch_off and covered[-1][1] == m.out.ch_off + m.K and \
                    all(a[1] == b[0] for a, b in zip(covered, covered[1:]))
                if not tiled or any(id(o) not in conv_ok for o in rd):
                    drop.add(id(u))
        if not drop:
            return [u for u in units if id(u) in eligible], dict(conv_ok.values())
        eligible -= drop


class Net:
    def __init__(self, batch, input_size=299, k=5, mode="train", fine_tune=False, device="cuda", seed=2,
                 bn_decay=0.9997, repeats=(10, 20, 9), bn_max_workgroups=0, wgrad_overlap_cus=None):
        assert mode in ("train", "infer")
        self.repeats = tuple(repeats)
        self.B, self.S, self.k, self.mode, self.fine_tune, self.dev = batch, input_size, k, mode, fine_tune, device
        self.bn_decay = bn_decay
        self.tune_registry = []
        self.deterministic = bool(int(os.environ.get("MBX_DETERMINISTIC", "0")))
        self.no_onepass = self.deterministic or bool(int(os.environ.get("MBX_NO_BN_ONEPASS", "0")))
        self.atomic_stats = mode == "train" and not self.deterministic and os.environ.get("MBX_ATOMIC_STATS", "1") != "0"
        self.bw_stats = self.atomic_stats and os.environ.get("MBX_BW_STATS", "0") == "1"
        self.fuse_apply = self.atomic_stats and os.environ.get("MBX_FUSE_APPLY", "0") == "1"
        self.fused_apply_launches = 0
        self.fuse_bwd = (mode == "train" and not self.deterministic and not self.bw_stats and torch.device(device).type == "cuda"
                         and os.environ.get("MBX_FUSE_BWD", "0") == "1")
        self.fused_bwd_launches = self.fused_bwd_layers = 0
        self.relu_bits = mode == "train" and os.environ.get("MBX_RELU_BITS", "1") != "0"
        self.autotune = torch.device(device).type == "cuda" and bool(int(os.environ.get("MBX_AUTOTUNE", "1")))
        self.bn_max_wg = int(os.environ.get("MBX_BN_MAX_WG", "0")) or (bn_max_workgroups or 0)
        self.wgrad_overlap_cus = ops.wgrad_overlap_cus() if wgrad_overlap_cus is None else int(wgrad_overlap_cus)
        self.n_cus = torch.cuda.get_device_properties(device).multi_processor_count if torch.device(device).type == "cuda" else 256
        self.chain_cap = 0
        if self.wgrad_overlap_cus > 0 and mode == "train":
            self.wgrad_overlap_cus = min(self.wgrad_overlap_cus, self.n_cus // 2)
            self.chain_cap = min(self.bn_max_wg or self.n_cus, self.n_cus - self.wgrad_overlap_cus)
        self.cu_cap = 0
        self.defer_moving = False
        self.i5_counters = torch.zeros(8192, dtype=torch.int32, device=device)
        self._i5_used = 0
        self._probe_skip_apply = self._probe_skip_bn_bwd = False
        self.convs, self.fwd, self.bwd = [], [], []
        self._bn_group_requests, self.bn_groups = [], []
        self.grad_alias = {}
        self.written = set()
        self.heads = []
        self._bufs = []
        self._keep = []
        self._build()
        self._finalize(seed)

    def alloc(self, H, W, Cc, dtype=torch.bfloat16, zero=False):
        v = View.alloc(self.B, H, W, Cc, dtype=dtype, device=self.dev, zero=zero)
        self._bufs.append(v.buf)
        return v

    def grad_of(self, v: View) -> View:
        key = id(v.buf)
        if key not in self.grad_alias:
            g = torch.zeros_like(v.buf)
            self._bufs.append(g)
            self.grad_alias[key] = g
        return View(self.grad_alias[key], v.N, v.H, v.W, v.C, v.ld, v.ch_off, v.elem_size)

    def share_grad(self, v: View, like: View):
        self.grad_alias[id(v.buf)] = self.grad_of(like).buf

    def _training_bn(self, is_head):
        if self.mode == "infer":
            return False
        return is_head if self.fine_tune else True
# ... 480 lines not shown
        if d.relu_bits and d.epilogue == ops.EPI_RESIDUAL:
            key = key + ("bits",)
        self.tune_registry.append((repr(key), d, what))
        if self.autotune:
            ops.autotune(d, key)
            over = ops._TUNED.get(repr(key) + "#norule") if os.environ.get("MBX_NO_RULE_EXCEPTIONS") != "1" else None
            if over is not None:
                keep = d.tile_config
                d.tile_config = int(over)
                if _lib.lib().mbx_conv_supported(C.byref(d)) != 0:
                    d.tile_config, over = keep, None
            if os.environ.get("MBX_NO_I5") == "1" and d.tile_config > ops.I5_FLAG:
                d.tile_config = ops._TUNED.get(repr(key) + "#i3", 0)
            if d.tile_config > ops.I5_FLAG and os.environ.get("MBX_I5_STATIC") != "1":
                n = ops.I7_COUNTERS if d.tile_config == ops.I7_TILE_CONFIG else 1
                assert self._i5_used + n <= self.i5_counters.numel()
                d.work_counter = self.i5_counters.data_ptr() + 4 * self._i5_used
                self._i5_used += n
            if os.environ.get("MBX_NO_2STAGE") == "1":
                d.tile_config = {9: 7, 10: 2, 11: 5, 12: 2, 13: 8, 14: 1}.get(d.tile_config, d.tile_config)
            pair = (what == "fwd" and bool(d.stats_partial) and op.group is not None and len(op.group.members) == 2
                    and os.environ.get("MBX_CONV_PAIR", "1") != "0")
            rule = ops.launch_rule(d, pair) if over is None else None
            if rule is not None:
                d.tile_config, d.work_counter = rule[0], None
                _lib.check(_lib.lib().mbx_conv_supported(C.byref(d)), rule[1] + " " + op.name)
        return d

    def _build_forward_launches(self):
        L = []
        l = _lib.lib()
        st = lambda: torch.cuda.current_stream().cuda_stream
        for op in self.fwd:
            if isinstance(op, PoolOp):
                if not op.fused_fwd:
                    L.append(op.forward)
                continue
            if op.kind == "bn":
                L.append(self._bn_forward(op))
            elif op.kind == "frozen":
                d = self._tune(op, self._desc(op, op.out, epilogue=ops.EPI_AFFINE, relu=op.relu,
                                              scale=self._sl(self.bn_scale, op.beta_off, op.K),
                                              shift=self._sl(self.bn_shift, op.beta_off, op.K)), "fwd")
                L.append(lambda d=d, op=op: _lib.check(l.mbx_conv(C.byref(d), st()), op.name))
            elif op.kind == "residual":
                d = self._tune(op, self._desc(op, op.out, epilogue=ops.EPI_RESIDUAL, relu=op.relu,
                                              shift=self._sl(self.W, op.b_off, op.K), skip=op.skip, rscale=op.rscale,
                                              relu_bits=op.relu_bits), "fwd")
                L.append(lambda d=d, op=op: _lib.check(l.mbx_conv(C.byref(d), st()), op.name))
            elif op.kind == "head":
                d = self._desc(op, op.out, epilogue=ops.EPI_STORE_F32)
                L.append(lambda d=d, op=op: _lib.check(l.mbx_conv(C.byref(d), st()), op.name))
                if op is self.heads[-1]:
                    L.append(lambda: _lib.check(l.mbx_head_gather_all(self.head_table, len(self.heads), self.B, self.P,
                                                                      self.locs.data_ptr(), self.logits.data_ptr(), st()), "head_gather_all"))
        return L

    def _bn_forward(self, op):
        l = _lib.lib()
        st = lambda: torch.cuda.current_stream().cuda_stream
        cuda = torch.device(self.dev).type == "cuda"
        u = op.unit
        i, n, single = u.members.index(op), len(u.members), len(u.members) == 1
        fpool = op.fused_pool
        use16 = self.atomic_stats and fpool is None
        if use16:
            d = self._desc(op, op.y_view, stats=self.stats16[op.stats16_off:], stats_rows_mod=STATS_ROWS, stats_ld=0 if single else u.K)
        else:
            d = self._desc(op, op.y_view, stats=self.stats_scratch[op.stats_off:])
        d = self._tune(op, d, "fwd")
        S_ = ops.splitk_slices(d, self.n_cus) if single and cuda else 0
        if S_:
            d.tile_config = ops.SPLITK_FLAG + S_
            need = int(l.mbx_conv_splitk_workspace_bytes(C.byref(d)))
            ws = torch.empty(need // 4, dtype=torch.float32, device=self.dev)
            self._keep.append(ws)
            d.splitk_ws, d.splitk_ws_bytes = ws.data_ptr(), ws.numel() * 4
            _lib.check(l.mbx_conv_supported(C.byref(d)), "split-K " + op.name)
        rows = u.rows[i] = ops.conv_stats_rows(d)
        assert use16 or i + 1 == n or rows * op.K * 2 <= u.stats_off[i + 1] - u.stats_off[i]
        u.fwd_desc[i] = d
        if i + 1 < n:
            return lambda: None if u.pair_fwd else _lib.check(l.mbx_conv(C.byref(d), st()), op.name)
        if n == 2 and cuda and os.environ.get("MBX_CONV_PAIR", "1") != "0":
            u.pair_fwd = l.mbx_conv_pair(C.byref(u.fwd_desc[0]), C.byref(d), st()) == 0
        K, M, out = u.K, op.M, op.out
        mean, rstd, mm, mv, var, beta, thr = (self._sl(t, u.lead.beta_off, K) for t in
                                              (self.bn_mean, self.bn_rstd, self.MM, self.MV, self.bn_var, self.Bt, self.bn_thr))
        s16 = self.stats16[u.stats16_base:]
        a_ptr, a_ld, amap = u.target([m.out for m in u.members])
        amap = None if amap is None else C.byref(amap)
        parts = (C.c_void_p * n)(*[self.stats_scratch.data_ptr() + 4 * o for o in u.stats_off])
        rows_a, cs_a = (C.c_int32 * n)(*u.rows), (C.c_int32 * n)(*[m.K for m in u.members])
        if fpool is not None:
            fpool.fused_fwd = True
        fd = ba = None
        if single and use16 and self.fuse_apply and not S_ and cuda and out.img_stride == out.H * out.W * out.ld \
                and (not os.environ.get("MBX_FUSE_APPLY_ONLY") or re.search(os.environ["MBX_FUSE_APPLY_ONLY"], op.name)):
            ba = ops.BnApplyDesc()
            ba.barrier = self._fwd_barrier_base + ops.GRID_BARRIER_BYTES * self._fwd_barriers_used
            ba.a, ba.ld_a, ba.beta, ba.mean, ba.rstd = out.ptr, out.ld, beta.data_ptr(), mean.data_ptr(), rstd.data_ptr()
            ba.relu_thr, ba.relu, ba.eps, ba.step_poison = thr.data_ptr(), int(op.relu), BN_EPS, self.step_ctl.data_ptr()
            fd = ops.ConvDesc.from_buffer_copy(d)
            fd.bn_apply = C.addressof(ba)
            fd.work_counter = None
            if l.mbx_conv_supported(C.byref(fd)) == 0:
                assert self._fwd_barriers_used < self._n_fwd_barriers
                self._fwd_barriers_used += 1
                self.fused_apply_launches += 1
# ... 138 lines not shown
                else:
                    pre = None
            else:
                dyv, scale, db = op.dy_view, 1.0, None
                pre = self._bn_backward(op)
            ddesc = fdesc = None
            if op.need_dx:
                gx = self._gview(op.x)
                acc, acc_src = self._claim(gx)
                dyin = View(dyv.buf, dyv.N, dyv.H, dyv.W, op.kpad, dyv.ld, dyv.ch_off, 2)
                mr = mask_of.get(id(op))
                ddesc = ops.make_desc(dyin, self.Wd[op.dgrad_off:], op.Cin, op.R, op.S, op.stride,
                                      op.R - 1 - op.pad_t, op.S - 1 - op.pad_l, gx, transposed=1, accumulate=acc,
                                      rscale=(scale if scale != 1.0 else 0.0), skip=(mr.out if mr is not None else None),
                                      acc_src=acc_src)
                if mr is not None and self.relu_bits and op.Cin % 8 == 0:
                    bits = torch.zeros((op.x.N * op.x.H * op.x.W, (op.Cin + 31) // 32 * 4), dtype=torch.uint8, device=self.dev)
                    alt = ops.make_desc(dyin, self.Wd[op.dgrad_off:], op.Cin, op.R, op.S, op.stride,
                                        op.R - 1 - op.pad_t, op.S - 1 - op.pad_l, gx, transposed=1, accumulate=acc,
                                        rscale=(scale if scale != 1.0 else 0.0), acc_src=acc_src, relu_bits=bits)
                    if torch.device(self.dev).type != "cuda" or l.mbx_conv_supported(C.byref(alt)) == 0:
                        ddesc, mr.relu_bits = alt, bits
                self._tune(op, ddesc, "dgrad")
                if op.fb_segments is not None:
                    assert acc == 0 and acc_src is None and mr is None, op.name
                    fdesc = ops.ConvDesc.from_buffer_copy(ddesc)
                    fdesc.bn_bwd = C.addressof(self._fb_table(op))
                    fdesc.work_counter = None
                    if not (ops.I5_FLAG < fdesc.tile_config <= ops.I5_FLAG + 7 or fdesc.tile_config in (ops.DIRECTW_TILE_CONFIG, ops.RESIDENT_TILE_CONFIG)):
                        fdesc.tile_config = ops.i5_tile_for(op.x.M, op.Cin, self.n_cus)
                    if l.mbx_conv_supported(C.byref(fdesc)) != 0:
                        fdesc.tile_config = ops.i5_tile_for(op.x.M, op.Cin, self.n_cus)
                    _lib.check(l.mbx_conv_supported(C.byref(fdesc)), "data gradient + BN backward " + op.name)
                    self.fused_bwd_launches += 1
                if op.bw_segments is not None:
                    assert acc == 0 and acc_src is None and mr is None, op.name
                    ddesc.bn_bwd_stats = C.addressof(self._bw_table(op))
                    if l.mbx_conv_supported(C.byref(ddesc)) != 0:
                        for alt in (ops.I5_TILE_CONFIGS[2], ops.I5_TILE_CONFIGS[1], 0):
                            ddesc.tile_config = alt
                            if alt == 0:
                                ddesc.work_counter = None
                            if l.mbx_conv_supported(C.byref(ddesc)) == 0:
                                break
                        _lib.check(l.mbx_conv_supported(C.byref(ddesc)), "statistics epilogue " + op.name)

            job = ops.WgradJob()
            job.desc = ops.make_desc(op.x, None, K, op.R, op.S, op.stride, op.pad_t, op.pad_l,
                                     View(dyv.buf, op.out.N, op.out.H, op.out.W, 8, dyv.ld, dyv.ch_off, 2))
            job.desc.C_out = K
            job.dy, job.dy_img_stride, job.ld_dy = dyv.ptr, dyv.img_stride, dyv.ld
            job.scale = float(scale)
            job.dw, job.db = dw.data_ptr(), (None if db is None else db.data_ptr())

            grp = op.group
            if grp is not None and ddesc is not None:
                grp.dgrad_desc[grp.members.index(op)] = ddesc

            op.fdesc = fdesc

            def run(op=op, pre=pre, ddesc=ddesc, grp=grp, fdesc=fdesc):
                s = st()
                if pre is not None and not (op.kind == "bn" and self._probe_skip_bn_bwd):
                    pre(s)
                if fdesc is not None and not self.no_onepass:
                    fdesc.max_workgroups = self.cu_cap or self.bn_max_wg
                    _lib.check(l.mbx_conv(C.byref(fdesc), s), "dgrad + bn backward " + op.name)
                    return
                if ddesc is not None:
                    if grp is not None and grp.pair_bwd:
                        if op is grp.members[-1]:
                            _lib.check(l.mbx_conv_pair(C.byref(ddesc), C.byref(grp.dgrad_desc[0]), s), "dgrad pair " + op.name)
                        return
                    ddesc.max_workgroups = self.cu_cap
                    _lib.check(l.mbx_conv(C.byref(ddesc), s), "dgrad " + op.name)
            L.append(run)
            self.bwd_ops.append(op)
            self.bwd_jobs.append(job)
        if torch.device(self.dev).type == "cuda" and os.environ.get("MBX_CONV_PAIR", "1") != "0":
            for grp in self.bn_groups:
                if len(grp.members) == 2 and len(grp.dgrad_desc) == 2 and not any(m.fdesc is not None for m in grp.members):
                    grp.pair_bwd = l.mbx_conv_pair(C.byref(grp.dgrad_desc[1]), C.byref(grp.dgrad_desc[0]), st()) == 0
        assert not self.pending_acc, "a residual block's input gradient was never written"
        self.bwd_launches = L
        self.fwd_launches = self._build_forward_launches()
        self._default_groups = None

    def _bn_backward(self, op):
        l = _lib.lib()
        u = op.unit
        if op is not u.members[-1]:
            return None
        K, M, relu, fpool = u.K, op.M, int(op.relu), op.fused_pool
        rows3 = l.mbx_bn_bwd_rows(M, K)
        y_ptr, dy_ptr, scratch, m12 = u.y.data_ptr(), u.dy.data_ptr(), self.bwd_scratch.data_ptr(), self.m12.data_ptr()
        mean, rstd, beta, dbeta, thr = (self._sl(t, u.lead.beta_off, K).data_ptr() for t in
                                        (self.bn_mean, self.bn_rstd, self.Bt, self.Btg, self.bn_thr))
        da_ptr = da_ld = dmap = None
        if fpool is None:
            da_ptr, da_ld, dmap = u.target([self._gview(m.out) for m in u.members])
            dmap = None if dmap is None else C.byref(dmap)

        def three(s):
            _lib.check(l.mbx_bn_bwd_reduce_mapped(da_ptr, da_ld, None, 0, relu, y_ptr, M, K, mean, rstd, beta, scratch, dmap, s),
                       "bn_bwd_reduce")
            _lib.check(l.mbx_bn_bwd_finalize(scratch, rows3, K, M, dbeta, m12, s), "bn_bwd_finalize")
            apply_only(s)

        def apply_only(s):
            _lib.check(l.mbx_bn_bwd_apply_mapped(da_ptr, da_ld, None, 0, relu, y_ptr, M, K, mean, rstd, beta, m12, dy_ptr, dmap, s),
                       "bn_bwd_apply")

        if fpool is not None:
            gy = self._gview(fpool.out)
            rows = l.mbx_bn_bwd_rows_pooled(fpool.x.N, fpool.x.H, fpool.x.W, K)
            assert 0 < rows * K * 2 <= self.bwd_scratch.numel()

            def form(s):
                geo = (gy.ptr, gy.img_stride, gy.ld, fpool.argmax.data_ptr(), fpool.x.N, fpool.x.H, fpool.x.W, fpool.out.H,
                       fpool.out.W, relu, y_ptr, K, mean, rstd, beta)
                _lib.check(l.mbx_bn_bwd_reduce_pooled(*geo, scratch, s), "bn_bwd_reduce_pooled")
                _lib.check(l.mbx_bn_bwd_finalize(scratch, rows, K, M, dbeta, m12, s), "bn_bwd_finalize")
                _lib.check(l.mbx_bn_bwd_apply_pooled(*geo, m12, dy_ptr, s), "bn_bwd_apply_pooled")
        elif op.bw_unit is not None:
            rows_ptr = self.bn_ws.data_ptr() + 4 * u.lead.bw_rows_off

            def form(s):
                _lib.check(l.mbx_bn_bwd_apply_rows(rows_ptr, STATS_ROWS, da_ptr, da_ld, y_ptr, M, K, mean, rstd, thr, dbeta,
                                                   dy_ptr, dmap, s), "bn_bwd_apply_rows")
        elif u.lead.bn_ws_off >= 0:
            ws_ptr = self.bn_ws.data_ptr() + 4 * u.lead.bn_ws_off

            def one(s):
                _lib.check(l.mbx_bn_bwd_onepass_mapped(da_ptr, da_ld, relu, y_ptr, M, K, mean, rstd, beta, dbeta, dy_ptr, ws_ptr,
                                                       self.cu_cap or self.bn_max_wg, self.step_ctl.data_ptr(), dmap, s),
                           "bn_bwd_onepass")

            def form(s):
                (three if self.no_onepass else one)(s)
            if os.environ.get("MBX_PROBE_BN_APPLY_ONLY") == "1":
                form = apply_only
        else:
            form = three
        if op.fb_unit is None:
            return form
        self.fused_bwd_layers += 1

        def unless_fused(s):
            if self.no_onepass:
                form(s)
        return unless_fused

    def _pool_producer(self, pool):
        if os.environ.get("MBX_POOL_FUSE", "1") == "0" or pool.kind != "max" or pool.k != 3 or pool.stride != 2 or pool.pad != 0 \
                or pool.argmax is None:
            return None
        readers = [o for o in self.fwd if o is not pool and o.x.buf is pool.x.buf]
        if readers:
            return None
        for c in self.convs:
            if c.out.buf is pool.x.buf and c.out.ch_off == pool.x.ch_off and c.out.C == pool.x.C and c.out.ld == pool.x.ld == pool.x.C:
                ok = c.kind == "bn" and c.trainable and c.group is None and (c.bn_ws_off < 0 or self.deterministic)
                return c if ok else None
        return None

    def make_wgrad_groups(self, job_lists):
        return [ops.WgradGroup(jobs, deterministic=self.deterministic, device=self.dev) for jobs in job_lists if jobs]

    def prepare_filters(self):
        if self.mode == "train" and self.filter_entries:
            _lib.check(_lib.lib().mbx_filter_prepare(self.Wb.data_ptr(), self.Wd.data_ptr(), self.filter_table.data_ptr(),
                                                     self.filter_entries, self.filter_blocks,
                                                     torch.cuda.current_stream().cuda_stream), "filter_prepare")

    def apply_moving_update(self, skip_ctl=None, skipped_steps=None, ema_mean=None, ema_var=None, ema_decay=0.0):
        lo = self.head_bt_start if self.fine_tune else 0
        n = self.nBt - lo
        if n > 0 and self.mode == "train":
            _lib.check(_lib.lib().mbx_bn_moving_update(self.MM.data_ptr() + 4 * lo, self.MV.data_ptr() + 4 * lo,
                                                       self.bn_mean.data_ptr() + 4 * lo, self.bn_var.data_ptr() + 4 * lo, n,
                                                       self.bn_decay, ops._p(skip_ctl), ops._p(skipped_steps),
                                                       None if ema_mean is None else ema_mean.data_ptr() + 4 * lo,
                                                       None if ema_var is None else ema_var.data_ptr() + 4 * lo, float(ema_decay),
                                                       torch.cuda.current_stream().cuda_stream), "bn_moving_update")

    def fold_bn(self):
        _lib.check(_lib.lib().mbx_bn_fold(self.MM.data_ptr(), self.MV.data_ptr(), self.Bt.data_ptr(), BN_EPS, self.nBt,
                                          self.bn_scale.data_ptr(), self.bn_shift.data_ptr(),
                                          torch.cuda.current_stream().cuda_stream), "bn_fold")

    def set_input(self, images_f32):
        assert images_f32.shape == (self.B, self.S, self.S, 3) and images_f32.dtype == torch.float32
        _lib.check(_lib.lib().mbx_pack_input(images_f32.contiguous().data_ptr(), self.B * self.S * self.S,
                                             self.images.buf.data_ptr(), torch.cuda.current_stream().cuda_stream), "pack_input")

    def forward(self):
        if self._i5_used or self.atomic_stats:
            self._fwd_clear.zero_()
        for f in self.fwd_launches:
            f()
        return self.locs, self.logits

    def layer_table(self):
        writers = {}

        def record(v: View, scope):
            lst = [w for w in writers.get(id(v.buf), []) if w[1] <= v.ch_off or w[0] >= v.ch_off + v.C]
            lst.append((v.ch_off, v.ch_off + v.C, scope))
            writers[id(v.buf)] = lst

        def producers(v: View):
            if v.buf is self.images.buf:
                return ["inputs"]
            inside = sorted(w for w in writers.get(id(v.buf), []) if w[0] >= v.ch_off and w[1] <= v.ch_off + v.C)
            assert inside and inside[0][0] == v.ch_off and inside[-1][1] == v.ch_off + v.C and \
                all(a[1] == b[0] for a, b in zip(inside, inside[1:])), "input view is not tiled by earlier outputs"
            return [w[2] for w in inside]

        table = []
        for op in self.fwd:
            if isinstance(op, PoolOp):
                table.append({"scope": op.scope, "op": op.kind + "_pool2d", "in_channels": op.x.C, "out_channels": op.out.C,
                              "kernel": [op.k, op.k], "stride": op.stride, "pad": [op.pad, op.pad],
                              "out_hw": [op.out.H, op.out.W], "inputs": producers(op.x)})
                record(op.out, op.scope)
                continue
            ins = producers(op.x)
            off = 0
            for m in op.members:
                e = {"scope": m.scope, "op": "conv2d", "in_channels": 3 if op.x.buf is self.images.buf else op.Cin,
                     "out_channels": m.K, "kernel": [op.R, op.S], "stride": op.stride, "pad": [op.pad_t, op.pad_l],
                     "out_hw": [op.out.H, op.out.W], "inputs": ins, "bn": op.kind in ("bn", "frozen"),
                     "bias": op.kind == "residual", "activation": "relu" if (op.relu and op.kind != "residual") else None}
                if op.kind == "residual":
                    e["residual"] = {"scale": op.rscale, "skip": producers(op.skip), "activation": "relu" if op.relu else None}
                table.append(e)
                if op.kind != "head":
                    record(op.out.slice(off, m.K), m.scope)
                off += m.K
        return table

    def flops_per_image(self, train=True):
        total = 0.0
        for op in self.convs:
            f = 2.0 * (op.M // self.B) * op.K * op.Cin * op.R * op.S
            total += f * (3.0 if (train and op.trainable) else 1.0)
        return total

    def barrier_timeouts(self):
        if self.mode != "train":
            return 0
        return int(self.bn_timeouts_total) + int(float(self.step_ctl[0]))

    def zero_grads(self):
        n_clear = self.G_off if self.fine_tune else self.G.numel()
        _lib.check(_lib.lib().mbx_step_begin(self.G.data_ptr(), n_clear, self.bn_ws.data_ptr(), self.bn_ws.numel(),
                                             self.nBt, self.bn_timeouts_total.data_ptr(), self.reg_loss.data_ptr(),
                                             torch.cuda.current_stream().cuda_stream), "step_begin")
        if self.fine_tune:
            self.Wg[self.head_w_start:].zero_()

    def backward(self):
        if self._i5_used:
            self.i5_counters.zero_()
        for f in self.bwd_launches:
            f()
        self.run_deferred_wgrad()

    def run_deferred_wgrad(self):
        if self._default_groups is None:
            jobs = [j for j in self.bwd_jobs if j is not None]
            n = max(1, (len(jobs) + 3) // 4)
            self._default_groups = self.make_wgrad_groups([jobs[i:i + n] for i in range(0, len(jobs), n)])
        for g in self._default_groups:
            g.launch()


class PoolOp:
    def __init__(self, net, kind, x: View, out: View, k, stride, pad):
        self.net, self.kind, self.x, self.out, self.k, self.stride, self.pad = net, kind, x, out, k, stride, pad
        self.argmax = None
        self.fused_fwd = False
        if kind == "max" and net.mode == "train" and not net.fine_tune:
            self.argmax = torch.zeros((out.N, out.H, out.W, out.C), dtype=torch.uint8, device=net.dev)

    def needs_backward(self):
        return self.net.mode == "train" and not self.net.fine_tune

    def forward(self):
        l, x, y = _lib.lib(), self.x, self.out
        s = torch.cuda.current_stream().cuda_stream
        if self.kind == "max":
            _lib.check(l.mbx_maxpool_fwd(x.ptr, x.img_stride, x.ld, x.N, x.H, x.W, x.C, self.k, self.stride, y.ptr,
                                         y.img_stride, y.ld, y.H, y.W, None if self.argmax is None else self.argmax.data_ptr(), s),
                       "maxpool_fwd")
        else:
            _lib.check(l.mbx_avgpool_fwd(x.ptr, x.img_stride, x.ld, x.N, x.H, x.W, x.C, self.k, self.pad, y.ptr,
                                         y.img_stride, y.ld, y.H, y.W, s), "avgpool_fwd")

    def make_backward(self, gy: View, gx: View, acc):
        l, x, y = _lib.lib(), self.x, self.out

        def run():
            s = torch.cuda.current_stream().cuda_stream
            if self.kind == "max":
                _lib.check(l.mbx_maxpool_bwd(gy.ptr, gy.img_stride, gy.ld, self.argmax.data_ptr(), x.N, x.H, x.W, x.C, self.k,
                                             self.stride, y.H, y.W, gx.ptr, gx.img_stride, gx.ld, acc, s), "maxpool_bwd")
            else:
                _lib.check(l.mbx_avgpool_bwd(gy.ptr, gy.img_stride, gy.ld, x.N, x.H, x.W, x.C, self.k, self.pad, y.H, y.W,
                                             gx.ptr, gx.img_stride, gx.ld, acc, s), "avgpool_bwd")
        return run
```

### multibox_amd/loss.py

```python
from __future__ import annotations

import ctypes

import torch

from . import _lib
from .config import LOC_LOSS_TYPES as LOC_TYPES

SMALL_EPSILON = 1e-10


def _stream():
    return torch.cuda.current_stream().cuda_stream


def _f32(t):
    assert t.is_cuda and t.dtype == torch.float32 and t.is_contiguous(), "expected contiguous float32 CUDA tensor"
    return t


def _i32(t):
    assert t.is_cuda and t.dtype == torch.int32 and t.is_contiguous(), "expected contiguous int32 CUDA tensor"
    return t

# ... 80 lines not shown
            raise ValueError("loc_beta is given without loc_loss")
        return None
    if not (isinstance(loc_loss, str) and loc_loss in LOC_TYPES):
        raise ValueError("loc_loss must be one of %s, got %r" % (", ".join(LOC_TYPES), loc_loss))
    if loc_loss != "smooth_l1":
        if loc_beta is not None:
            raise ValueError("loc_beta goes with loc_loss 'smooth_l1' only, got it with %r" % (loc_loss,))
        return LOC_TYPES.index(loc_loss), 0.0
    if loc_beta is None:
        return LOC_TYPES.index(loc_loss), LOC_BETA_DEFAULT
    if not (isinstance(loc_beta, (int, float)) and not isinstance(loc_beta, bool)
            and 0.0 < ctypes.c_float(loc_beta).value < float("inf")):
        raise ValueError("loc_beta must be a finite number > 0 (as a float32), got %r" % (loc_beta,))
    return LOC_TYPES.index(loc_loss), float(loc_beta)


class MultiboxLoss:

    def __init__(self, bbox_priors, batch_size, max_num_bboxes, location_loss_alpha, device="cuda", neg_per_pos=None,
                 min_neg=0, match_iou_threshold=None, focal_gamma=None, focal_alpha=None, loc_loss=None, loc_beta=None,
                 atss_topk=None, prior_levels=None):
        self.focal = _focal_arguments(focal_gamma, focal_alpha)
        self.loc = _loc_arguments(loc_loss, loc_beta)
        self.priors = torch.as_tensor(bbox_priors, dtype=torch.float32).to(device).contiguous()
        self.P = self.priors.shape[0]
        self.B, self.G, self.alpha = int(batch_size), int(max_num_bboxes), float(location_loss_alpha)
        f = dict(dtype=torch.float32, device=device)
        self.decoded = torch.empty((self.B, self.P, 4), **f)
        self.conf = torch.empty((self.B, self.P), **f)
        self.match = torch.empty((self.B, self.P), dtype=torch.int32, device=device)
        self.status = torch.zeros((self.B,), dtype=torch.int32, device=device)
        self.loss2 = torch.zeros((2,), **f)
        self.d_locs = torch.empty((self.B, self.P, 4), **f)
        self.d_logits = torch.empty((self.B, self.P), **f)
        self.neg_per_pos, self.min_neg, self.n_neg = neg_per_pos, min_neg, None
        mining = (0, 0, None)
        if neg_per_pos is not None:
            self.n_neg = torch.zeros((self.B,), dtype=torch.int32, device=device)
            mining = (neg_per_pos, min_neg, self.n_neg.data_ptr())
        l = _lib.lib()
        if self.loc is not None:
            self.entry, self.entry_args = "mbx_loss_fwd_bwd_loc", self.loc + (self.focal or (0.0, 1.0, 1.0)) + mining
            ws_bytes = l.mbx_loss_loc_workspace_bytes(self.B, self.P)
        elif self.focal is not None:
            self.entry, self.entry_args = "mbx_loss_fwd_bwd_focal", self.focal + mining
            ws_bytes = l.mbx_loss_focal_workspace_bytes(self.B, self.P)
        elif neg_per_pos is not None:
            self.entry, self.entry_args = "mbx_loss_fwd_bwd_mined", mining
            ws_bytes = l.mbx_loss_mined_workspace_bytes(self.B, self.P)
        else:
            self.entry, self.entry_args = "mbx_loss_fwd_bwd", ()
            ws_bytes = l.mbx_loss_workspace_bytes(self.B)
        self.ws = torch.empty((ws_bytes,), dtype=torch.uint8, device=device)
        self.match_iou_threshold, self.n_extra = match_iou_threshold, None
        if match_iou_threshold is not None:
            if not 0.0 < float(match_iou_threshold) <= 1.0:
                raise ValueError("match_iou_threshold must be in (0, 1], got %r" % (match_iou_threshold,))
            self.match_iou_threshold = float(match_iou_threshold)
            self.n_extra = torch.zeros((self.B,), dtype=torch.int32, device=device)
        self.atss_topk, self.prior_levels, self.n_atss, self.atss_thr = None, None, None, None
        if atss_topk is not None:
            if match_iou_threshold is not None:
                raise ValueError("atss_topk and match_iou_threshold are both given: each decides what a free prior becomes")
            if not (isinstance(atss_topk, int) and not isinstance(atss_topk, bool) and 1 <= atss_topk <= 2 ** 31 - 1):
                raise ValueError("atss_topk must be an int >= 1, got %r" % (atss_topk,))
            if prior_levels is None:
                raise ValueError("atss_topk needs prior_levels, the list [0, ..., P] of where each level of the priors starts")
            try:
                levels = [int(v) for v in prior_levels]
            except (TypeError, ValueError):
                raise ValueError("prior_levels must be a list of ints, got %r" % (prior_levels,))
            if not (2 <= len(levels) <= 9 and levels[0] == 0 and levels[-1] == self.P
                    and all(a < b for a, b in zip(levels, levels[1:]))):
                raise ValueError("prior_levels must hold 1 to 8 levels, start at 0, ascend strictly and end at the %d priors, "
                                 "got %r" % (self.P, levels))
            self._level_table, self._n_levels = _level_table(levels)
            verdict = l.mbx_match_atss_supported(self.P, self.G, self._n_levels, self._level_table, atss_topk)
            if verdict != 0:
                raise ValueError("atss_topk %d with prior_levels %r, %d priors and %d boxes an image: mbx_match_atss says %s"
                                 % (atss_topk, levels, self.P, self.G, l.mbx_status_string(verdict).decode()))
            self.atss_topk, self.prior_levels = atss_topk, levels
            self.n_atss = torch.zeros((self.B,), dtype=torch.int32, device=device)
            self.atss_thr = torch.zeros((self.B, self.G), dtype=torch.float64, device=device)
        elif prior_levels is not None:
            raise ValueError("prior_levels is given without atss_topk")

    def forward_backward(self, raw_locs, logits, gt_bboxes, num_gt_bboxes, grad_scale=1.0, conf_is_logit=True):
        l, s = _lib.lib(), _stream()
        B, P, G = self.B, self.P, self.G
        assert raw_locs.shape == (B, P, 4) and logits.numel() == B * P and gt_bboxes.shape == (B, G, 4)
        if conf_is_logit:
            _lib.check(l.mbx_decode_conf(_f32(raw_locs).data_ptr(), _f32(logits).data_ptr(), self.priors.data_ptr(),
                                         B, P, SMALL_EPSILON, self.decoded.data_ptr(), self.conf.data_ptr(), s),
                       "mbx_decode_conf")
        else:
            _lib.check(l.mbx_decode_conf(_f32(raw_locs).data_ptr(), None, self.priors.data_ptr(), B, P, 0.0,
                                         self.decoded.data_ptr(), None, s), "mbx_decode_conf")
            torch.add(logits.reshape(B, P), SMALL_EPSILON, out=self.conf)
        _lib.check(l.mbx_match(self.decoded.data_ptr(), self.conf.data_ptr(), _f32(gt_bboxes).data_ptr(),
                               _i32(num_gt_bboxes).data_ptr(), self.alpha, B, P, G, self.match.data_ptr(),
                               self.status.data_ptr(), None, 0, s), "mbx_match")
        if self.match_iou_threshold is not None:
            _lib.check(l.mbx_match_extend(self.priors.data_ptr(), gt_bboxes.data_ptr(), num_gt_bboxes.data_ptr(),
                                          self.status.data_ptr(), self.match_iou_threshold, B, P, G,
                                          self.match.data_ptr(), self.n_extra.data_ptr(), s), "mbx_match_extend")
        if self.atss_topk is not None:
            _lib.check(l.mbx_match_atss(self.priors.data_ptr(), self._level_table, self._n_levels, gt_bboxes.data_ptr(),
                                        num_gt_bboxes.data_ptr(), self.status.data_ptr(), self.atss_topk, B, P, G,
                                        self.match.data_ptr(), self.n_atss.data_ptr(), self.atss_thr.data_ptr(), s),
                       "mbx_match_atss")
        common = (self.decoded.data_ptr(), _f32(logits).data_ptr(), int(bool(conf_is_logit)), gt_bboxes.data_ptr(),
                  self.match.data_ptr(), self.alpha, float(grad_scale), B, P, G, self.loss2.data_ptr(), self.d_locs.data_ptr(),
                  self.d_logits.data_ptr())
        _lib.check(getattr(l, self.entry)(*common, *self.entry_args, self.ws.data_ptr(), self.ws.numel(), s), self.entry)
        return self.loss2, self.d_locs, self.d_logits


def add_loss(locations, confidences, batched_bboxes, batched_num_bboxes, bbox_priors, location_loss_alpha):
    B = locations.shape[0]
    m = MultiboxLoss(bbox_priors, B, batched_bboxes.shape[1], location_loss_alpha, device=locations.device)
    loss2, _, _ = m.forward_backward(locations.contiguous(), confidences.reshape(B, -1).contiguous(),
                                     batched_bboxes.to(torch.float32).contiguous(),
                                     batched_num_bboxes.to(torch.int32).contiguous(), conf_is_logit=False)
    st = m.status.cpu()
    if int(st.max()) != 0:
        raise ValueError("add_loss: matching failed (status %s)" % st.tolist())
    return loss2[0].clone(), loss2[1].clone()
```

### multibox_amd/ops.py

```python
from __future__ import annotations

import ctypes as C
import os

import torch

from . import _lib

EPI_STORE, EPI_AFFINE, EPI_RESIDUAL, EPI_STORE_F32 = 0, 1, 2, 3


class ConvDesc(C.Structure):
    _fields_ = [
        ("x", C.c_void_p), ("x_img_stride", C.c_int64), ("ldx", C.c_int32),
        ("N", C.c_int32), ("H_in", C.c_int32), ("W_in", C.c_int32), ("C_in", C.c_int32),
        ("w", C.c_void_p), ("C_out", C.c_int32), ("R", C.c_int32), ("S", C.c_int32),
        ("stride", C.c_int32), ("transposed", C.c_int32), ("pad_t", C.c_int32), ("pad_l", C.c_int32),
        ("H_out", C.c_int32), ("W_out", C.c_int32),
        ("y", C.c_void_p), ("y_img_stride", C.c_int64), ("ldy", C.c_int32),
        ("epilogue", C.c_int32), ("relu", C.c_int32), ("accumulate", C.c_int32),
        ("scale", C.c_void_p), ("shift", C.c_void_p),
        ("skip", C.c_void_p), ("skip_img_stride", C.c_int64), ("ld_skip", C.c_int32), ("rscale", C.c_float),
        ("stats_partial", C.c_void_p),
        ("tile_config", C.c_int32),
# ... 319 lines not shown
        if t < best_t * 0.97 or (cfg == 0 and t < best_t):
            best, best_t = cfg, t
    desc.tile_config = best
    _TUNED[key] = best
    return best


def autotune_wgrad(desc: ConvDesc, dy: View, scale, dw, db, key, candidates=(0, 2, 3, 4, 7, 8, 9, 10), iters=10):
    key = repr(key)
    if key in _TUNED:
        desc.tile_config = _TUNED[key]
        return desc.tile_config
    l = _lib.lib()
    s = _stream()
    best, best_t = 0, float("inf")
    iters = int(os.environ.get("MBX_TUNE_ITERS", iters))
    if os.environ.get("MBX_AUTOTUNE_WG"):
        candidates = tuple(int(v) for v in os.environ["MBX_AUTOTUNE_WG"].split(","))
    args = (dy.ptr, dy.img_stride, dy.ld, float(scale), dw.data_ptr(), _p(db), s)
    for cfg in candidates:
        desc.tile_config = cfg
        if l.mbx_conv_wgrad_scaled(C.byref(desc), *args) != 0:
            continue
        e0, e1 = torch.cuda.Event(enable_timing=True), torch.cuda.Event(enable_timing=True)
        e0.record()
        for _ in range(iters):
            l.mbx_conv_wgrad_scaled(C.byref(desc), *args)
        e1.record()
        e1.synchronize()
        t = e0.elapsed_time(e1)
        if t < best_t * 0.97 or (cfg == 0 and t < best_t):
            best, best_t = cfg, t
    desc.tile_config = best
    _TUNED[key] = best
    return best


class WgradGroup:

    def __init__(self, jobs, deterministic=False, device="cuda"):
        l = _lib.lib()
        self.n = len(jobs)
        arr = (WgradJob * self.n)(*jobs)
        flags = (1 if deterministic else 0) | (2 if os.environ.get("MBX_WGRAD_SCATTER") == "1" else 0)
        nbytes = l.mbx_wgrad_plan_bytes(arr, self.n, flags)
        assert nbytes > 0
        host = (C.c_uint8 * nbytes)()
        self.info = WgradPlanInfo()
        _lib.check(l.mbx_wgrad_plan(arr, self.n, flags, host, nbytes, C.byref(self.info)), "mbx_wgrad_plan")
        import numpy as np
        self.host_image = np.frombuffer(host, dtype=np.uint8).copy()
        self.image = torch.from_numpy(self.host_image).to(device)
        self.flops = float(self.info.flops)

    def launch(self, max_workgroups=0):
        _lib.check(_lib.lib().mbx_conv_wgrad_grouped_capped(self.image.data_ptr(), C.byref(self.info), int(max_workgroups),
                                                            _stream()), "mbx_conv_wgrad_grouped")

    def tally(self):
        o = int(self.info.tally_off)
        t = self.image[o:o + 16].cpu().numpy().view("<u8")
        return int(t[0]), int(t[1])

    def completed_ok(self):
        items, launches = self.tally()
        return items == launches * int(self.info.n_items)

    def reset(self):
        self.image.copy_(torch.from_numpy(self.host_image))
```

### multibox_amd/trainer.py

```python
from __future__ import annotations

import math
import os
import re

import torch

from . import _lib
from .config import check_optimizer_args, check_trust_args
from .engine import Net, WEIGHT_DECAY
from .loss import MultiboxLoss
from .dist import BucketReducer


def decay_steps(num_train_examples, batch_size, num_epochs_per_decay):
    return int((int(num_train_examples) // int(batch_size)) * num_epochs_per_decay)


def learning_rate(step, lr0, dsteps, factor, staircase=True):
    p = step / float(dsteps)
    if staircase:
        p = math.floor(p)
    return float(lr0) * float(factor) ** p


def warmup_factor(step, warmup_steps):
    return min(1.0, (step + 1.0) / warmup_steps) if warmup_steps else 1.0


class Trainer:
    def __init__(self, net: Net, bbox_priors, max_num_bboxes=13, location_loss_alpha=1000.0, initial_learning_rate=0.01,
                 decay_steps_=7116, learning_rate_decay_factor=0.94, staircase=True, rmsprop_decay=0.9,
                 rmsprop_momentum=0.0, rmsprop_epsilon=1.0, moving_average_decay=0.9999, use_graph=True,
                 n_segments=None, process_group=None, trainable_scopes=None, neg_per_pos=None, min_neg=0,
                 match_iou_threshold=None, focal_gamma=None, focal_alpha=None, loc_loss=None, loc_beta=None,
                 clip_gradient_norm=None, optimizer="rmsprop", sgd_momentum=0.9, sgd_nesterov=False, adam_beta1=0.9,
                 adam_beta2=0.999, adam_epsilon=1e-8, adamw_weight_decay=0.01, lr_warmup_steps=0, atss_topk=None,
                 layerwise_trust=False, trust_coeff=None):
        assert net.mode == "train"
        self.net = net
        self.pg = process_group
        prior_levels = None if atss_topk is None else [op.head[2] for op in net.heads] + [net.P]
        self.loss = MultiboxLoss(bbox_priors, net.B, max_num_bboxes, location_loss_alpha, device=net.dev,
                                 neg_per_pos=neg_per_pos, min_neg=min_neg, match_iou_threshold=match_iou_threshold,
                                 focal_gamma=focal_gamma, focal_alpha=focal_alpha, loc_loss=loc_loss, loc_beta=loc_beta,
                                 atss_topk=atss_topk, prior_levels=prior_levels)
        assert self.loss.P == net.P, "priors (%d) do not match the network's predictions (%d)" % (self.loss.P, net.P)
        self.loss.d_locs, self.loss.d_logits = net.d_locs, net.d_logits
        self.lr0, self.dsteps, self.lr_factor, self.staircase = initial_learning_rate, decay_steps_, learning_rate_decay_factor, staircase
        self.rms_decay, self.momentum, self.eps, self.ema_decay = rmsprop_decay, rmsprop_momentum, rmsprop_epsilon, moving_average_decay
        self.global_step = 0
        self.reducer = BucketReducer(process_group)
        f32 = dict(dtype=torch.float32, device=net.dev)
        self.w_lo = net.head_w_start if net.fine_tune else 0
        self.bt_lo = net.head_bt_start if net.fine_tune else 0
        self.optimizer = optimizer or "rmsprop"
        check_optimizer_args(self.optimizer, sgd_momentum, adam_beta1, adam_beta2, adam_epsilon, adamw_weight_decay)
        self.trust_coeff = check_trust_args(self.optimizer, layerwise_trust, trust_coeff)
        self.sgd_momentum, self.sgd_nesterov = float(sgd_momentum), bool(sgd_nesterov)
        self.adam_beta1, self.adam_beta2, self.adam_eps = float(adam_beta1), float(adam_beta2), float(adam_epsilon)
        self.wd_decoupled = float(adamw_weight_decay) if self.optimizer == "adamw" else 0.0
        self.wd_l2 = 0.0 if self.optimizer == "adamw" else WEIGHT_DECAY
        self.warmup_steps = int(lr_warmup_steps or 0)
        self._opt_step_offset = 0
        has_mom = {"rmsprop": self.momentum != 0.0, "sgd": self.sgd_momentum != 0.0}.get(self.optimizer, True)
        second = None if self.optimizer == "sgd" else torch.ones if self.optimizer == "rmsprop" else torch.zeros
        self.Wms = second(net.nW, **f32) if second else None
        self.Btms = second(net.nBt, **f32) if second else None
        self.Wmom = torch.zeros(net.nW, **f32) if has_mom else None
        self.Btmom = torch.zeros(net.nBt, **f32) if has_mom else None
        self.Wema, self.Btema = net.W.clone(), net.Bt.clone()
        self.MMema, self.MVema = net.MM.clone(), net.MV.clone()
        self.frozen_reg = 0.0
        self.refresh_frozen_reg()
        self.opt_ranges = self._optimizer_ranges(trainable_scopes)
        self._trust_plans = None if self.trust_coeff is None else {
            i: self._trust_plan(lo, hi) for i, (buf, lo, hi, on) in enumerate(self.opt_ranges) if buf == "W" and on and hi > lo}
        self.gt = torch.zeros((net.B, max_num_bboxes, 4), **f32)
        self.n_gt = torch.zeros((net.B,), dtype=torch.int32, device=net.dev)
        self.images = torch.zeros((net.B, net.S, net.S, 3), **f32)
        net.prepare_filters()
        if net.fine_tune:
            net.fold_bn()
        self.use_graph = use_graph
        self.graphs = None
        self.events = []
        self._timeouts_seen = 0
        self._stop_flag = torch.zeros((), **f32)
        net.defer_moving = True
        self.skipped_steps = torch.zeros((), dtype=torch.int64, device=net.dev)
        self._skipped_seen = 0
        self.clip_norm = None
        if clip_gradient_norm is not None:
            self.clip_norm = float(clip_gradient_norm)
            if not self.clip_norm > 0:
                raise ValueError("clip_gradient_norm must be > 0 (inf = guard only), got %r" % (clip_gradient_norm,))
            slots = _lib.lib().mbx_grad_sqnorm_partials
            self._clip_slots = [(int(slots(hi - lo)) if on and hi > lo else 0) for _, lo, hi, on in self.opt_ranges]
            self._clip_partials = torch.zeros((max(1, sum(self._clip_slots)),), dtype=torch.float64, device=net.dev)
            self._clip_block = torch.zeros((8,), **f32)
            self._clip_block[2] = 1.0
# ... 174 lines not shown
                raise RuntimeError("batch-norm backward: %d grid-barrier timeout(s) AFTER the fall-back to the three-launch form" % t)
            import sys
            net.no_onepass = True
            self.graphs = None
            self.events.append({"event": "bn_backward_fallback", "global_step": self.global_step, "barrier_timeouts": t})
            print("[multibox_amd] step %d: %d grid-barrier timeout(s) in the one-launch BN backward (workgroups not co-resident); "
                  "the affected steps were NOT applied; continuing with the three-launch BN backward" % (self.global_step, t),
                  file=sys.stderr)
            out["fallback"] = True
            return out
        if m:
            raise RuntimeError("bipartite matching failed on %d rank(s) (non-finite predictions or n_gt > P)" % m)
        if w:
            for g in self.wgrad_groups:
                g.reset()
            raise RuntimeError("grouped weight gradient: %d launch group(s) did not process all their work items "
                               "(queue heads re-uploaded)" % w)
        return out

    def _make_segments(self, n, tail_params=0, by_work=False):
        net = self.net
        tagged = list(zip(net.bwd_launches, net.bwd_ops, net.bwd_jobs))
        from .engine import PoolOp
        total = net.nW - self.w_lo
        target = max(total // max(n, 1), 1)

        def work(job):
            d = job.desc
            return float(d.N) * d.H_out * d.W_out * d.C_out * d.R * d.S * d.C_in
        wtarget = max(sum(work(j) for j in net.bwd_jobs if j is not None) / max(n, 1), 1.0)
        wacc = 0.0
        segs, cur, jobs, hi = [], [], [], net.nW
        lo = hi
        for fn, op, job in tagged:
            cur.append(fn)
            if job is not None:
                jobs.append(job)
                wacc += work(job)
            if not isinstance(op, PoolOp):
                lo = min(lo, op.w_off)
                full = (wacc >= wtarget * (len(segs) + 1)) if by_work else (hi - lo >= target)
                if full and hi > lo and len(segs) < n - 1:
                    segs.append((cur, lo, hi, jobs))
                    cur, jobs, hi = [], [], lo
                elif tail_params > 0 and len(segs) == n - 1 and hi > lo and 0 < lo - self.w_lo <= tail_params:
                    segs.append((cur, lo, hi, jobs))
                    cur, jobs, hi = [], [], lo
                    tail_params = 0
        if cur:
            segs.append((cur, self.w_lo, hi, jobs))
        on_gpu = torch.device(net.dev).type == "cuda"
        groups = net.make_wgrad_groups([j for _, _, _, j in segs]) if on_gpu else []
        self.wgrad_groups = groups
        self._seg_groups, gi = [], 0
        for _, _, _, jobs in segs:
            if jobs and on_gpu:
                self._seg_groups.append(groups[gi])
                gi += 1
            else:
                self._seg_groups.append(None)
        return [(fns, lo, hi) for fns, lo, hi, _ in segs]

    def _run_segment(self, i):
        for f in self._segments[i][0]:
            f()
        if self._seg_groups[i] is not None:
            self._seg_groups[i].launch()

    def _front(self):
        net = self.net
        first = net.fuse_apply
        if first:
            net.zero_grads()
        net.set_input(self.images)
        net.forward()
        self.loss.forward_backward(net.locs, net.logits, self.gt, self.n_gt)
        if not first:
            net.zero_grads()

    def _capture(self):
        net = self.net
        self._front_merged = False
        mm, mv = net.MM.clone(), net.MV.clone()
        self._front()
        for i in range(len(self._segments)):
            self._run_segment(i)
        net.MM.copy_(mm)
        net.MV.copy_(mv)
        torch.cuda.synchronize()
        graphs = []
        nseg, K = len(self._segments), self.overlap_cus
        mode = dict(capture_error_mode="thread_local")
        if K and self._side is None:
            self._side = torch.cuda.Stream()

        def chain(i, capped):
            net.cu_cap = net.chain_cap if capped else 0
            try:
                for f in self._segments[i][0]:
                    f()
            finally:
                net.cu_cap = 0

        def beside(fn):
            self._side.wait_stream(torch.cuda.current_stream())
            with torch.cuda.stream(self._side):
                fn()
            forked[0] = True

        def join():
            if forked[0]:
                torch.cuda.current_stream().wait_stream(self._side)
                forked[0] = False
        forked = [False]
        if K and not self.reducer.enabled:
            g = torch.cuda.CUDAGraph()
            with torch.cuda.graph(g, **mode):
                self._front()
                for i in range(nseg):
                    chain(i, capped=i > 0)
                    grp = self._seg_groups[i]
                    if grp is None:
                        continue
                    if i == nseg - 1:
                        join()
                        grp.launch()
                    else:
                        beside(lambda grp=grp: grp.launch(K))
                join()
# ... 195 lines not shown
```

Baseline: 4394 images/sec.

## Fold loss finalize, fuse gather+decode, register-resident matcher, and partial grad clears

Several independent changes to the train step. The head gather is fused with the prior decode. Zeroing of the forward buffers is folded into the input pack kernel. The loss kernels finish the cross-batch reduction themselves with an atomic ticket, so no separate finalize launch is needed. Gradient zeroing is limited to the ranges that weight-gradient groups accumulate into rather than the whole buffer, and a new register-resident Hungarian matcher with DPP wave reductions is added. Each change removes small launches or memory traffic, at the cost of more complex correctness invariants, such as the assertion that the cleared ranges match the default wgrad groups.

```diff
diff --git a/include/mbx.h b/include/mbx.h
--- a/include/mbx.h
+++ b/include/mbx.h
@@ -89,6 +89,17 @@
                          float gamma, float w_pos, float w_neg,
                          int neg_per_pos , int min_neg, int32_t* n_neg ,
                          void* workspace, size_t workspace_bytes, mbx_stream_t stream);
+
+enum { MBX_LOSS_PLAIN = 0, MBX_LOSS_MINED = 1, MBX_LOSS_FOCAL = 2, MBX_LOSS_LOC = 3 };
+size_t mbx_loss_folded_workspace_bytes(int B);
+int mbx_loss_fwd_bwd_folded(int kind , const float* decoded , const float* conf_in ,
+                            int conf_is_logit, const float* gt ,
+                            const int32_t* match , float alpha, float grad_scale, int B, int P,
+                            int G, float* loss2 ,
+                            float* d_raw_locs , float* d_logits ,
+                            int loc_type, float loc_beta, float gamma, float w_pos, float w_neg,
+                            int neg_per_pos, int min_neg, int32_t* n_neg ,
+                            void* workspace, size_t workspace_bytes, mbx_stream_t stream);
 
 typedef struct {
   int32_t offset_y, offset_x;
@@ -341,6 +352,7 @@
 
 int mbx_relu_mask(void* g, int ld_g, const void* a, int ld_a, int64_t M, int C, mbx_stream_t stream);
 int mbx_pack_input(const float* img, int64_t pixels, void* out, mbx_stream_t stream);
+int mbx_pack_input_clear(const float* img, int64_t pixels, void* out, int32_t* clear, int64_t n_clear, mbx_stream_t stream);
 int mbx_head_gather(const float* h, int ld_h, int N, int cells, int k, int P, int off,
                     float* locs, float* logits, mbx_stream_t stream);
 int mbx_head_scatter(const float* d_locs, const float* d_logits, int N, int cells, int k, int P,
@@ -355,9 +367,14 @@
                         mbx_stream_t stream);
 int mbx_head_scatter_all(const float* d_locs, const float* d_logits, const mbx_head* heads , int n_heads, int N,
                          int P, mbx_stream_t stream);
+int mbx_head_gather_decode(const mbx_head* heads , int n_heads, int N, int P, const float* priors, float eps_add,
+                           float* locs, float* logits, float* decoded, float* conf, mbx_stream_t stream);
 
 int mbx_step_begin(float* grads, int64_t n_grads, float* bn_ws, int64_t n_ws, int64_t ctl_index, uint64_t* timeouts_total,
                    float* zero_scalar, mbx_stream_t stream);
+int mbx_step_begin_ranges(float* grads, int64_t n_grads, int64_t n_head, const int64_t* ranges ,
+                          int n_ranges, int64_t range_elems, float* bn_ws, int64_t n_ws, int64_t ctl_index,
+                          uint64_t* timeouts_total, float* zero_scalar, mbx_stream_t stream);
 
 typedef struct {
   int64_t src_off;
diff --git a/multibox_amd/_lib.py b/multibox_amd/_lib.py
--- a/multibox_amd/_lib.py
+++ b/multibox_amd/_lib.py
@@ -39,6 +39,8 @@
     "mbx_loss_fwd_bwd_focal": (I, [P, P, I, P, P, F, F, I, I, I, P, P, P, F, F, F, I, I, P, P, SZ, P]),
     "mbx_loss_loc_workspace_bytes": (SZ, [I, I]),
     "mbx_loss_fwd_bwd_loc": (I, [P, P, I, P, P, F, F, I, I, I, P, P, P, I, F, F, F, F, I, I, P, P, SZ, P]),
+    "mbx_loss_folded_workspace_bytes": (SZ, [I]),
+    "mbx_loss_fwd_bwd_folded": (I, [I, P, P, I, P, P, F, F, I, I, I, P, P, P, I, F, F, F, F, I, I, P, P, SZ, P]),
     "mbx_decode_filter_topk": (I, [P, P, P, P, I, I, I, P, P, P, P, P]),
     "mbx_nms": (I, [P, P, P, P, I, I, C.c_double, P]),
     "mbx_merge_detections": (I, [P, P, P, P, I, I, I, C.c_double, P, P, P, P, P, P]),
@@ -90,6 +92,9 @@
     "mbx_avgpool_bwd": (I, [P, C.c_int64, I, I, I, I, I, I, I, I, I, P, C.c_int64, I, I, P]),
     "mbx_relu_mask": (I, [P, I, P, I, C.c_int64, I, P]),
     "mbx_pack_input": (I, [P, C.c_int64, P, P]),
+    "mbx_pack_input_clear": (I, [P, C.c_int64, P, P, C.c_int64, P]),
+    "mbx_head_gather_decode": (I, [P, I, I, I, P, F, P, P, P, P, P]),
+    "mbx_step_begin_ranges": (I, [P, C.c_int64, C.c_int64, P, I, C.c_int64, P, C.c_int64, C.c_int64, P, P, P]),
     "mbx_head_gather": (I, [P, I, I, I, I, I, I, P, P, P]),
     "mbx_head_scatter": (I, [P, P, I, I, I, I, I, P, I, P]),
     "mbx_head_gather_all": (I, [P, I, I, I, P, P, P]),
diff --git a/multibox_amd/csrc/loss.hip b/multibox_amd/csrc/loss.hip
--- a/multibox_amd/csrc/loss.hip
+++ b/multibox_amd/csrc/loss.hip
@@ -19,6 +19,36 @@
       conf[i] = __fadd_rn(s, eps_add);
     }
   }
+}
+
+template <int CTRL, int ROW_MASK>
+__device__ __forceinline__ void atss_dpp_min(unsigned long long& k) {
+  const unsigned olo = (unsigned)__builtin_amdgcn_update_dpp(-1, (int)(unsigned)k, CTRL, ROW_MASK, 0xf, false);
+  const unsigned ohi = (unsigned)__builtin_amdgcn_update_dpp(-1, (int)(unsigned)(k >> 32), CTRL, ROW_MASK, 0xf, false);
+  const unsigned long long ok = ((unsigned long long)ohi << 32) | olo;
+  if (ok < k) k = ok;
+}
+template <int CTRL, int ROW_MASK>
+__device__ __forceinline__ void atss_dpp_min(int& i) {
+  const int oi = __builtin_amdgcn_update_dpp(0x7fffffff, i, CTRL, ROW_MASK, 0xf, false);
+  if (oi < i) i = oi;
+}
+template <int CTRL, int ROW_MASK>
+__device__ __forceinline__ void atss_dpp_min(double& d) {
+  const unsigned long long k = (unsigned long long)__double_as_longlong(d);
+  const unsigned olo = (unsigned)__builtin_amdgcn_update_dpp(0, (int)(unsigned)k, CTRL, ROW_MASK, 0xf, false);
+  const unsigned ohi = (unsigned)__builtin_amdgcn_update_dpp(0x7ff00000, (int)(unsigned)(k >> 32), CTRL, ROW_MASK, 0xf, false);
+  const double o = __longlong_as_double((long long)(((unsigned long long)ohi << 32) | olo));
+  if (o < d) d = o;
+}
+template <typename T>
+__device__ __forceinline__ void atss_dpp_min_to_lane63(T& v) {
+  atss_dpp_min<0x111, 0xf>(v);
+  atss_dpp_min<0x112, 0xf>(v);
+  atss_dpp_min<0x114, 0xf>(v);
+  atss_dpp_min<0x118, 0xf>(v);
+  atss_dpp_min<0x142, 0xa>(v);
+  atss_dpp_min<0x143, 0xc>(v);
 }
 
 __device__ __forceinline__ double match_cost(const float4 l, const float4 g, float half_alpha,
@@ -183,6 +213,168 @@
   if (tid == 0) status[b] = 0;
 }
 
+struct WaveBest { double val; int key, pad; };
+constexpr int kKeyNone = 0x7fffffff, kKeyAssigned = 1 << 30;
+
+template <int NT, int CPL>
+__global__ void __launch_bounds__(NT)
+match_reg_kernel(const float4* __restrict__ decoded, const float* __restrict__ conf,
+                 const float4* __restrict__ gt, const int* __restrict__ n_gt, float alpha, int P, int G,
+                 int* __restrict__ match, int* __restrict__ status) {
+  extern __shared__ __attribute__((aligned(16))) unsigned char smem[];
+  float4* gts = reinterpret_cast<float4*>(smem);
+  double* spc_s = reinterpret_cast<double*>(gts + G);
+  double* u = spc_s + P;
+  int* path_s = reinterpret_cast<int*>(u + G);
+  int* row4col = path_s + P;
+  int* col4row = row4col + P;
+  int* SR = col4row + G;
+  constexpr int kNW = NT / 64;
+  __shared__ WaveBest wave_best[2][kNW];
+  __shared__ int sh_bad;
+
+  const int b = blockIdx.x, tid = threadIdx.x;
+  const float4* loc_g = decoded + (size_t)b * P;
+  const float* cf = conf + (size_t)b * P;
+  const float4* g = gt + (size_t)b * G;
+  int* mt = match + (size_t)b * P;
+  const int n = n_gt[b];
+  const float half_alpha = alpha / 2.0f;
+
+  float4 loc[CPL];
+  float lc[CPL], l1c[CPL];
+  double v[CPL], spc[CPL];
+  int path[CPL];
+  unsigned outside = 0u, unassigned = 0u;
+
+  if (tid == 0) sh_bad = 0;
+  __syncthreads();
+  int bad = 0;
+#pragma unroll
+  for (int c = 0; c < CPL; ++c) {
+    const int j = tid + c * NT;
+    loc[c] = make_float4(0.f, 0.f, 0.f, 0.f); lc[c] = 0.f; l1c[c] = 0.f; v[c] = 0.0; spc[c] = INFINITY; path[c] = 0;
+    if (j >= P) { outside |= 1u << c; continue; }
+    mt[j] = -1;
+    const float cc = cf[j];
+    lc[c] = logf(cc);
+    float w = __fsub_rn(1.0f, cc);
+    if (w > 1.0f) w = 1.0f;
+    if (w <= 0.0f) w = 1e-10f;
+    l1c[c] = logf(w);
+    row4col[j] = -1;
+    unassigned |= 1u << c;
+    const float4 l = loc_g[j];
+    loc[c] = l;
+    if (!(isfinite(lc[c]) && isfinite(l1c[c]) && isfinite(l.x) && isfinite(l.y) && isfinite(l.z) && isfinite(l.w))) bad = 1;
+  }
+  for (int i = tid; i < G; i += NT) {
+    u[i] = 0.0;
+    col4row[i] = -1;
+    float4 q = make_float4(0.f, 0.f, 0.f, 0.f);
+    if (i < n) {
+      q = g[i];
+      if (!(isfinite(q.x) && isfinite(q.y) && isfinite(q.z) && isfinite(q.w))) bad = 1;
+    }
+    gts[i] = q;
+  }
+  if (bad) sh_bad = 1;
+  __syncthreads();
+  if (n <= 0) { if (tid == 0) status[b] = 0; return; }
+  if (n > P || n > G) { if (tid == 0) status[b] = 1; return; }
+  if (sh_bad) { if (tid == 0) status[b] = 2; return; }
+
+  int it = 0;
+  for (int cur = 0; cur < n; ++cur) {
+    unsigned sc = outside;
+#pragma unroll
+    for (int c = 0; c < CPL; ++c) spc[c] = INFINITY;
+    for (int i = tid; i < n; i += NT) SR[i] = 0;
+    int i = cur, sink = -1, scans = 0;
+    double min_val = 0.0;
+    while (true) {
+      const float4 gi = gts[i];
+      const double ui = u[i];
+      double bval = INFINITY;
+      int bkey = kKeyNone;
+#pragma unroll
+      for (int c = 0; c < CPL; ++c) {
+        if (sc & (1u << c)) continue;
+        const double r = ((min_val + match_cost(loc[c], gi, half_alpha, lc[c], l1c[c])) - ui) - v[c];
+        if (r < spc[c]) { path[c] = i; spc[c] = r; }
+        const int key = (tid + c * NT) | ((unassigned & (1u << c)) ? 0 : kKeyAssigned);
+        if (bkey == kKeyNone || spc[c] < bval || (spc[c] == bval && key < bkey)) { bval = spc[c]; bkey = key; }
+      }
+      double wmin = bval;
+      atss_dpp_min_to_lane63(wmin);
+      wmin = __longlong_as_double((long long)(((unsigned long long)(unsigned)__builtin_amdgcn_readlane((int)((unsigned long long)__double_as_longlong(wmin) >> 32), 63) << 32) |
+                                              (unsigned)__builtin_amdgcn_readlane((int)(unsigned)__double_as_longlong(wmin), 63)));
+      unsigned long long tied = __ballot(bval == wmin);
+      if (__popcll(tied) > 1) {
+        int k = bval == wmin ? bkey : kKeyNone;
+        int kmin = k;
+        atss_dpp_min_to_lane63(kmin);
+        kmin = __builtin_amdgcn_readlane(kmin, 63);
+        tied = __ballot(k == kmin);
+      }
+      const int src = __ffsll((long long)tied) - 1;
+      if ((tid & 63) == src) {
+        WaveBest wb; wb.val = bval; wb.key = bkey; wb.pad = 0;
+        wave_best[it & 1][tid >> 6] = wb;
+      }
+      __syncthreads();
+      WaveBest bb = wave_best[it & 1][0];
+#pragma unroll
+      for (int w = 1; w < kNW; ++w) {
+        const WaveBest o = wave_best[it & 1][w];
+        if (o.val < bb.val || (o.val == bb.val && o.key < bb.key)) bb = o;
+      }
+      ++it;
+      if (bb.key == kKeyNone || !(bb.val < INFINITY) || ++scans > P) { sink = -2; break; }
+      min_val = bb.val;
+      const int bj = bb.key & (kKeyAssigned - 1);
+#pragma unroll
+      for (int c = 0; c < CPL; ++c)
+        if (tid + c * NT == bj) sc |= 1u << c;
+      if (tid == 0) SR[i] = 1;
+      if (!(bb.key & kKeyAssigned)) { sink = bj; break; }
+      i = row4col[bj];
+    }
+    if (sink == -2) { if (tid == 0) status[b] = 2; return; }
+#pragma unroll
+    for (int c = 0; c < CPL; ++c) {
+      if (!(sc & ~outside & (1u << c))) continue;
+      const int j = tid + c * NT;
+      spc_s[j] = spc[c];
+      path_s[j] = path[c];
+      v[c] -= min_val - spc[c];
+    }
+    __syncthreads();
+    for (int r = tid; r < n; r += NT) {
+      if (r == cur) u[r] += min_val;
+      else if (SR[r]) u[r] += min_val - spc_s[col4row[r]];
+    }
+    __syncthreads();
+    if (tid == 0) {
+      int j = sink;
+      for (int steps = 0; steps <= cur; ++steps) {
+        const int r = path_s[j];
+        row4col[j] = r;
+        const int t = col4row[r];
+        col4row[r] = j;
+        j = t;
+        if (r == cur) break;
+      }
+    }
+    __syncthreads();
+#pragma unroll
+    for (int c = 0; c < CPL; ++c)
+      if ((sc & ~outside & (1u << c)) && row4col[tid + c * NT] >= 0) unassigned &= ~(1u << c);
+  }
+  for (int i = tid; i < n; i += NT) mt[col4row[i]] = i;
+  if (tid == 0) status[b] = 0;
+}
+
 struct StagedBox { Box box; double area; };
 
 __global__ void __launch_bounds__(1024)
@@ -255,28 +447,6 @@
 
 __device__ __forceinline__ bool atss_pair_less(unsigned long long ka, int ia, unsigned long long kb, int ib) {
   return ka < kb || (ka == kb && ia < ib);
-}
-
-template <int CTRL, int ROW_MASK>
-__device__ __forceinline__ void atss_dpp_min(unsigned long long& k) {
-  const unsigned olo = (unsigned)__builtin_amdgcn_update_dpp(-1, (int)(unsigned)k, CTRL, ROW_MASK, 0xf, false);
-  const unsigned ohi = (unsigned)__builtin_amdgcn_update_dpp(-1, (int)(unsigned)(k >> 32), CTRL, ROW_MASK, 0xf, false);
-  const unsigned long long ok = ((unsigned long long)ohi << 32) | olo;
-  if (ok < k) k = ok;
-}
-template <int CTRL, int ROW_MASK>
-__device__ __forceinline__ void atss_dpp_min(int& i) {
-  const int oi = __builtin_amdgcn_update_dpp(0x7fffffff, i, CTRL, ROW_MASK, 0xf, false);
-  if (oi < i) i = oi;
-}
-template <typename T>
-__device__ __forceinline__ void atss_dpp_min_to_lane63(T& v) {
-  atss_dpp_min<0x111, 0xf>(v);
-  atss_dpp_min<0x112, 0xf>(v);
-  atss_dpp_min<0x114, 0xf>(v);
-  atss_dpp_min<0x118, 0xf>(v);
-  atss_dpp_min<0x142, 0xa>(v);
-  atss_dpp_min<0x143, 0xc>(v);
 }
 
 __device__ __forceinline__ void atss_wave_min(unsigned long long& k, int& i) {
@@ -630,7 +800,8 @@
                                           float grad_scale, int P, int G, int loc_type, float loc_beta, float gamma,
                                           float w_pos, float w_neg, int neg_per_pos, int min_neg,
                                           double* __restrict__ partial , float4* __restrict__ d_locs,
-                                          float* __restrict__ d_logits, int* __restrict__ n_neg) {
+                                          float* __restrict__ d_logits, int* __restrict__ n_neg,
+                                          unsigned* __restrict__ ticket, float* __restrict__ loss2) {
   constexpr bool kCountPositives = FOCAL && !MINED;
   const int b = blockIdx.x, tid = threadIdx.x;
   unsigned long long cut = 0ull;
@@ -689,36 +860,67 @@
     red[tid >> 6][0] = loc_acc; red[tid >> 6][1] = conf_acc;
     if (kCountPositives) pos_waves[tid >> 6] = n_pos;
   }
+  __shared__ int sh_last;
   __syncthreads();
   if (tid == 0) {
     double a = 0.0, c = 0.0;
     for (int w = 0; w < kWaves; ++w) { a += red[w][0]; c += red[w][1]; }
-    partial[2 * b] = a;
-    partial[2 * b + 1] = c;
+    if (!ticket) {
+      partial[2 * b] = a;
+      partial[2 * b + 1] = c;
+    } else {
+      __hip_atomic_store(partial + 2 * b, a, __ATOMIC_RELAXED, __HIP_MEMORY_SCOPE_AGENT);
+      __hip_atomic_store(partial + 2 * b + 1, c, __ATOMIC_RELAXED, __HIP_MEMORY_SCOPE_AGENT);
+      asm volatile("s_waitcnt vmcnt(0)" ::: "memory");
+      sh_last = atomicAdd(ticket, 1u) == gridDim.x - 1u;
+    }
     if (kCountPositives && n_neg) {
       int total = 0;
       for (int w = 0; w < kWaves; ++w) total += pos_waves[w];
       n_neg[b] = P - total;
     }
   }
+  if (!ticket) return;
+  __syncthreads();
+  if (!sh_last) return;
+  __shared__ double fin[2 * kThreads];
+  const int B = (int)gridDim.x;
+  for (int i = tid; i < 2 * B && i < 2 * kThreads; i += kThreads)
+    fin[i] = __hip_atomic_load(partial + i, __ATOMIC_RELAXED, __HIP_MEMORY_SCOPE_AGENT);
+  __syncthreads();
+  if (tid == 0) {
+    double a = 0.0, c = 0.0;
+    for (int i = 0; i < B; ++i) {
+      if (i < kThreads) { a += fin[2 * i]; c += fin[2 * i + 1]; }
+      else {
+        a += __hip_atomic_load(partial + 2 * i, __ATOMIC_RELAXED, __HIP_MEMORY_SCOPE_AGENT);
+        c += __hip_atomic_load(partial + 2 * i + 1, __ATOMIC_RELAXED, __HIP_MEMORY_SCOPE_AGENT);
+      }
+    }
+    const double loc_factor = (!LOC_ANY || loc_type == MBX_LOC_L2) ? 0.5 : 1.0;
+    loss2[0] = alpha * (float)(a * loc_factor);
+    loss2[1] = (float)c;
+    __hip_atomic_store(ticket, 0u, __ATOMIC_RELAXED, __HIP_MEMORY_SCOPE_AGENT);
+  }
 }
 
 __global__ void __launch_bounds__(kThreads)
 loss_kernel(const float4* __restrict__ decoded, const float* __restrict__ logits, int is_logit,
             const float4* __restrict__ gt, const int* __restrict__ match, float alpha, float grad_scale,
             int P, int G, double* __restrict__ partial , float4* __restrict__ d_locs,
-            float* __restrict__ d_logits) {
+            float* __restrict__ d_logits, unsigned* __restrict__ ticket, float* __restrict__ loss2) {
   loss_body<false, false, false>(decoded, logits, is_logit, gt, match, alpha, grad_scale, P, G, MBX_LOC_L2, 0.0f, 0.0f, 1.0f,
-                                 1.0f, 0, 0, partial, d_locs, d_logits, nullptr);
+                                 1.0f, 0, 0, partial, d_locs, d_logits, nullptr, ticket, loss2);
 }
 
 __global__ void __launch_bounds__(kThreads)
 loss_mined_kernel(const float4* __restrict__ decoded, const float* __restrict__ logits, int is_logit,
                   const float4* __restrict__ gt, const int* __restrict__ match, float alpha, float grad_scale,
                   int P, int G, int neg_per_pos, int min_neg, double* __restrict__ partial ,
-                  float4* __restrict__ d_locs, float* __restrict__ d_logits, int* __restrict__ n_neg) {
+                  float4* __restrict__ d_locs, float* __restrict__ d_logits, int* __restrict__ n_neg,
+                  unsigned* __restrict__ ticket, float* __restrict__ loss2) {
   loss_body<true, false, false>(decoded, logits, is_logit, gt, match, alpha, grad_scale, P, G, MBX_LOC_L2, 0.0f, 0.0f, 1.0f,
-                                1.0f, neg_per_pos, min_neg, partial, d_locs, d_logits, n_neg);
+                                1.0f, neg_per_pos, min_neg, partial, d_locs, d_logits, n_neg, ticket, loss2);
 }
 
 template <bool MINED>
@@ -727,9 +929,9 @@
                   const float4* __restrict__ gt, const int* __restrict__ match, float alpha, float grad_scale,
                   int P, int G, float gamma, float w_pos, float w_neg, int neg_per_pos, int min_neg,
                   double* __restrict__ partial , float4* __restrict__ d_locs, float* __restrict__ d_logits,
-                  int* __restrict__ n_neg) {
+                  int* __restrict__ n_neg, unsigned* __restrict__ ticket, float* __restrict__ loss2) {
   loss_body<MINED, true, false>(decoded, logits, is_logit, gt, match, alpha, grad_scale, P, G, MBX_LOC_L2, 0.0f, gamma, w_pos,
-                                w_neg, neg_per_pos, min_neg, partial, d_locs, d_logits, n_neg);
+                                w_neg, neg_per_pos, min_neg, partial, d_locs, d_logits, n_neg, ticket, loss2);
 }
 
 template <bool MINED>
@@ -738,9 +940,10 @@
                 const float4* __restrict__ gt, const int* __restrict__ match, float alpha, float grad_scale,
                 int P, int G, int loc_type, float loc_beta, float gamma, float w_pos, float w_neg, int neg_per_pos,
                 int min_neg, double* __restrict__ partial , float4* __restrict__ d_locs,
-                float* __restrict__ d_logits, int* __restrict__ n_neg) {
+                float* __restrict__ d_logits, int* __restrict__ n_neg, unsigned* __restrict__ ticket,
+                float* __restrict__ loss2) {
   loss_body<MINED, true, true>(decoded, logits, is_logit, gt, match, alpha, grad_scale, P, G, loc_type, loc_beta, gamma, w_pos,
-                               w_neg, neg_per_pos, min_neg, partial, d_locs, d_logits, n_neg);
+                               w_neg, neg_per_pos, min_neg, partial, d_locs, d_logits, n_neg, ticket, loss2);
 }
 
 }
@@ -763,6 +966,34 @@
 
 static size_t match_lds_bytes(int P, int G) { return (size_t)P * 36 + (size_t)G * 16 + 16; }
 
+constexpr int kMatchRegMaxP = 8 * 512;
+static size_t match_reg_lds_bytes(int P, int G) { return (size_t)P * 16 + (size_t)G * 32; }
+
+template <int NT, int CPL>
+static int launch_match_reg_as(const float* decoded, const float* conf, const float* gt, const int32_t* n_gt, float alpha,
+                               int B, int P, int G, int32_t* match, int32_t* status, hipStream_t s) {
+  const size_t lds = match_reg_lds_bytes(P, G);
+  if (lds > 60 * 1024) {
+    if (hipFuncSetAttribute(reinterpret_cast<const void*>(match_reg_kernel<NT, CPL>),
+                            hipFuncAttributeMaxDynamicSharedMemorySize, (int)lds) != hipSuccess) return MBX_ERR_LAUNCH;
+  }
+  hipLaunchKernelGGL((match_reg_kernel<NT, CPL>), dim3(B), dim3(NT), lds, s, reinterpret_cast<const float4*>(decoded), conf,
+                     reinterpret_cast<const float4*>(gt), n_gt, alpha, P, G, match, status);
+  return MBX_OK;
+}
+
+static int launch_match_reg(int nthreads, const float* decoded, const float* conf, const float* gt, const int32_t* n_gt,
+                            float alpha, int B, int P, int G, int32_t* match, int32_t* status, hipStream_t s) {
+  const int cpl = (P + nthreads - 1) / nthreads;
+#define MBX_MATCH_REG(NT, CPL) \
+  if (nthreads == NT && cpl == CPL) return launch_match_reg_as<NT, CPL>(decoded, conf, gt, n_gt, alpha, B, P, G, match, status, s);
+  MBX_MATCH_REG(256, 1) MBX_MATCH_REG(256, 2) MBX_MATCH_REG(256, 3) MBX_MATCH_REG(256, 4) MBX_MATCH_REG(256, 5)
+  MBX_MATCH_REG(256, 6) MBX_MATCH_REG(512, 4) MBX_MATCH_REG(512, 5) MBX_MATCH_REG(512, 6) MBX_MATCH_REG(512, 7)
+  MBX_MATCH_REG(512, 8)
+#undef MBX_MATCH_REG
+  return MBX_ERR_UNSUPPORTED;
+}
+
 extern "C" size_t mbx_match_workspace_bytes(int, int, int) { return 0; }
 
 extern "C" int mbx_match(const float* decoded, const float* conf, const float* gt, const int32_t* n_gt,
@@ -775,6 +1006,12 @@
   static const int force_nt = mbx_env_int("MBX_MATCH_THREADS", 0);
   const int nthreads = force_nt ? force_nt : (P > 1536 ? 512 : kThreads);
   MBX_ENTER();
+  if (!force_nt && P <= kMatchRegMaxP && match_reg_lds_bytes(P, G) <= 150 * 1024) {
+    const int st = launch_match_reg(nthreads, decoded, conf, gt, n_gt, alpha, B, P, G, match, status, mbx_s(stream));
+    if (st != MBX_OK) return st;
+    MBX_LAUNCH_CHECK();
+    return MBX_OK;
+  }
   if (lds > 64 * 1024) {
     if (hipFuncSetAttribute(reinterpret_cast<const void*>(match_kernel), hipFuncAttributeMaxDynamicSharedMemorySize,
                             (int)lds) != hipSuccess) return MBX_ERR_LAUNCH;
@@ -853,6 +1090,7 @@
 extern "C" size_t mbx_loss_mined_workspace_bytes(int B, int) { return mbx_loss_workspace_bytes(B); }
 extern "C" size_t mbx_loss_focal_workspace_bytes(int B, int) { return mbx_loss_workspace_bytes(B); }
 extern "C" size_t mbx_loss_loc_workspace_bytes(int B, int) { return mbx_loss_workspace_bytes(B); }
+extern "C" size_t mbx_loss_folded_workspace_bytes(int B) { return mbx_loss_workspace_bytes(B) + 16; }
 
 enum class LossKind { kPlain, kMined, kFocal, kLoc };
 
@@ -860,10 +1098,12 @@
                        const int32_t* match, float alpha, float grad_scale, int B, int P, int G, float* loss2,
                        float* d_raw_locs, float* d_logits, int loc_type, float loc_beta, float gamma, float w_pos,
                        float w_neg, int neg_per_pos, int min_neg, int32_t* n_neg, void* workspace, size_t workspace_bytes,
-                       mbx_stream_t stream) {
+                       mbx_stream_t stream, bool folded = false) {
   if (!decoded || !logits || !gt || !match || !loss2 || B <= 0 || P <= 0 || G <= 0) return MBX_ERR_INVALID_ARG;
-  if (!workspace || workspace_bytes < mbx_loss_workspace_bytes(B)) return MBX_ERR_WORKSPACE;
+  if (!workspace || workspace_bytes < (folded ? mbx_loss_folded_workspace_bytes(B) : mbx_loss_workspace_bytes(B)))
+    return MBX_ERR_WORKSPACE;
   double* partial = reinterpret_cast<double*>(workspace);
+  unsigned* ticket = folded ? reinterpret_cast<unsigned*>(partial + 2 * (size_t)B) : nullptr;
   const float4* dec4 = reinterpret_cast<const float4*>(decoded);
   const float4* gt4 = reinterpret_cast<const float4*>(gt);
   float4* dl4 = reinterpret_cast<float4*>(d_raw_locs);
@@ -871,24 +1111,25 @@
   switch (kind) {
     case LossKind::kPlain:
       hipLaunchKernelGGL(loss_kernel, dim3(B), dim3(kThreads), 0, mbx_s(stream), dec4, logits, conf_is_logit, gt4, match,
-                         alpha, grad_scale, P, G, partial, dl4, d_logits);
+                         alpha, grad_scale, P, G, partial, dl4, d_logits, ticket, loss2);
       break;
     case LossKind::kMined:
       hipLaunchKernelGGL(loss_mined_kernel, dim3(B), dim3(kThreads), 0, mbx_s(stream), dec4, logits, conf_is_logit, gt4,
-                         match, alpha, grad_scale, P, G, neg_per_pos, min_neg, partial, dl4, d_logits, n_neg);
+                         match, alpha, grad_scale, P, G, neg_per_pos, min_neg, partial, dl4, d_logits, n_neg, ticket, loss2);
       break;
     case LossKind::kFocal:
       hipLaunchKernelGGL(neg_per_pos ? loss_focal_kernel<true> : loss_focal_kernel<false>, dim3(B), dim3(kThreads), 0,
                          mbx_s(stream), dec4, logits, conf_is_logit, gt4, match, alpha, grad_scale, P, G, gamma, w_pos,
-                         w_neg, neg_per_pos, min_neg, partial, dl4, d_logits, n_neg);
+                         w_neg, neg_per_pos, min_neg, partial, dl4, d_logits, n_neg, ticket, loss2);
       break;
     case LossKind::kLoc:
       hipLaunchKernelGGL(neg_per_pos ? loss_loc_kernel<true> : loss_loc_kernel<false>, dim3(B), dim3(kThreads), 0,
                          mbx_s(stream), dec4, logits, conf_is_logit, gt4, match, alpha, grad_scale, P, G, loc_type, loc_beta,
-                         gamma, w_pos, w_neg, neg_per_pos, min_neg, partial, dl4, d_logits, n_neg);
+                         gamma, w_pos, w_neg, neg_per_pos, min_neg, partial, dl4, d_logits, n_neg, ticket, loss2);
       break;
   }
   MBX_LAUNCH_CHECK();
+  if (folded) return MBX_OK;
   hipLaunchKernelGGL(loss_final_kernel, dim3(1), dim3(64), 0, mbx_s(stream), partial, B, alpha,
                      loc_type == MBX_LOC_L2 ? 0.5 : 1.0, loss2);
   MBX_LAUNCH_CHECK();
@@ -942,3 +1183,34 @@
                      d_raw_locs, d_logits, loc_type, loc_beta, gamma, w_pos, w_neg, neg_per_pos, min_neg, n_neg, workspace,
                      workspace_bytes, stream);
 }
+
+extern "C" int mbx_loss_fwd_bwd_folded(int kind, const float* decoded, const float* logits, int conf_is_logit,
+                                       const float* gt, const int32_t* match, float alpha, float grad_scale, int B, int P,
+                                       int G, float* loss2, float* d_raw_locs, float* d_logits, int loc_type, float loc_beta,
+                                       float gamma, float w_pos, float w_neg, int neg_per_pos, int min_neg, int32_t* n_neg,
+                                       void* workspace, size_t workspace_bytes, mbx_stream_t stream) {
+  switch (kind) {
+    case MBX_LOSS_PLAIN:
+      return launch_loss(LossKind::kPlain, decoded, logits, conf_is_logit, gt, match, alpha, grad_scale, B, P, G, loss2,
+                         d_raw_locs, d_logits, MBX_LOC_L2, 0.0f, 0.0f, 1.0f, 1.0f, 0, 0, nullptr, workspace, workspace_bytes,
+                         stream, true);
+    case MBX_LOSS_MINED:
+      if (neg_per_pos < 1 || min_neg < 0) return MBX_ERR_INVALID_ARG;
+      return launch_loss(LossKind::kMined, decoded, logits, conf_is_logit, gt, match, alpha, grad_scale, B, P, G, loss2,
+                         d_raw_locs, d_logits, MBX_LOC_L2, 0.0f, 0.0f, 1.0f, 1.0f, neg_per_pos, min_neg, n_neg, workspace,
+                         workspace_bytes, stream, true);
+    case MBX_LOSS_FOCAL:
+      if (!focal_arguments_ok(gamma, w_pos, w_neg, neg_per_pos, min_neg)) return MBX_ERR_INVALID_ARG;
+      return launch_loss(LossKind::kFocal, decoded, logits, conf_is_logit, gt, match, alpha, grad_scale, B, P, G, loss2,
+                         d_raw_locs, d_logits, MBX_LOC_L2, 0.0f, gamma, w_pos, w_neg, neg_per_pos, min_neg, n_neg, workspace,
+                         workspace_bytes, stream, true);
+    case MBX_LOSS_LOC:
+      if (loc_type < MBX_LOC_L2 || loc_type > MBX_LOC_CIOU) return MBX_ERR_INVALID_ARG;
+      if (loc_type == MBX_LOC_SMOOTH_L1 && !(loc_beta > 0.0f && !isinf(loc_beta))) return MBX_ERR_INVALID_ARG;
+      if (!focal_arguments_ok(gamma, w_pos, w_neg, neg_per_pos, min_neg)) return MBX_ERR_INVALID_ARG;
+      return launch_loss(LossKind::kLoc, decoded, logits, conf_is_logit, gt, match, alpha, grad_scale, B, P, G, loss2,
+                         d_raw_locs, d_logits, loc_type, loc_beta, gamma, w_pos, w_neg, neg_per_pos, min_neg, n_neg, workspace,
+                         workspace_bytes, stream, true);
+  }
+  return MBX_ERR_INVALID_ARG;
+}
diff --git a/multibox_amd/csrc/nnops.hip b/multibox_amd/csrc/nnops.hip
--- a/multibox_amd/csrc/nnops.hip
+++ b/multibox_amd/csrc/nnops.hip
@@ -289,7 +289,9 @@
 }
 
 __global__ void __launch_bounds__(kT)
-pack_input_kernel(const float* __restrict__ img, long long pixels, unsigned short* __restrict__ out) {
+pack_input_kernel(const float* __restrict__ img, long long pixels, unsigned short* __restrict__ out,
+                  int* __restrict__ clear, long long n_clear) {
+  for (long long i = (long long)blockIdx.x * kT + threadIdx.x; i < n_clear; i += (long long)gridDim.x * kT) clear[i] = 0;
   for (long long i = (long long)blockIdx.x * kT + threadIdx.x; i < pixels; i += (long long)gridDim.x * kT) {
     float f[8] = {img[3 * i], img[3 * i + 1], img[3 * i + 2], 0.f, 0.f, 0.f, 0.f, 0.f};
     st8(out + 8 * i, pack8(f));
@@ -343,6 +345,30 @@
     const size_t p = (size_t)n * P + t.off[j] + cell * k + a;
     *reinterpret_cast<float4*>(locs + p * 4) = make_float4(row[a * 4], row[a * 4 + 1], row[a * 4 + 2], row[a * 4 + 3]);
     logits[p] = row[4 * k + a];
+  }
+}
+
+__global__ void __launch_bounds__(kT)
+head_gather_all_decode_kernel(const HeadTable t, int P, const float4* __restrict__ priors, float eps_add,
+                              float* __restrict__ locs, float* __restrict__ logits, float4* __restrict__ decoded,
+                              float* __restrict__ conf) {
+  const int total = t.start[t.n];
+  for (int i = blockIdx.x * kT + threadIdx.x; i < total; i += gridDim.x * kT) {
+    int j = 0;
+    while (j + 1 < t.n && i >= t.start[j + 1]) ++j;
+    const int e = i - t.start[j], k = t.k[j], cells = t.cells[j];
+    const int a = e % k, q = e / k, cell = q % cells, n = q / cells;
+    const float* row = t.h[j] + (size_t)(n * cells + cell) * t.ld_h[j];
+    const int pp = t.off[j] + cell * k + a;
+    const size_t p = (size_t)n * P + pp;
+    const float4 r = make_float4(row[a * 4], row[a * 4 + 1], row[a * 4 + 2], row[a * 4 + 3]);
+    const float z = row[4 * k + a];
+    *reinterpret_cast<float4*>(locs + p * 4) = r;
+    logits[p] = z;
+    const float4 pr = priors[pp];
+    decoded[p] = make_float4(__fadd_rn(r.x, pr.x), __fadd_rn(r.y, pr.y), __fadd_rn(r.z, pr.z), __fadd_rn(r.w, pr.w));
+    const float s = 1.0f / (1.0f + expf(-z));
+    conf[p] = __fadd_rn(s, eps_add);
   }
 }
 
@@ -377,6 +403,42 @@
       reinterpret_cast<float4*>(G)[i] = z;
     } else {
       reinterpret_cast<float4*>(ws)[i - n4] = z;
+    }
+  }
+}
+
+__global__ void __launch_bounds__(kT)
+step_begin_ranges_kernel(float* __restrict__ G, long long nG, long long n_head, const long long* __restrict__ ranges,
+                         int n_ranges, float* __restrict__ ws, long long nws, long long ctl,
+                         unsigned long long* __restrict__ timeouts_total, float* __restrict__ scalar) {
+  if (scalar && blockIdx.x == 0 && threadIdx.x == 0) *scalar = 0.f;
+  const long long n4 = n_head >> 2, w4 = nws >> 2;
+  const long long gid = (long long)blockIdx.x * kT + threadIdx.x, gsz = (long long)gridDim.x * kT;
+  const float4 z = make_float4(0.f, 0.f, 0.f, 0.f);
+  for (long long i = gid; i < n4 + w4; i += gsz) {
+    if (i < n4) {
+      if (timeouts_total && i == (ctl >> 2)) {
+        const float t = G[ctl];
+        if (t > 0.f) *timeouts_total += (unsigned long long)t;
+      }
+      reinterpret_cast<float4*>(G)[i] = z;
+    } else {
+      reinterpret_cast<float4*>(ws)[i - n4] = z;
+    }
+  }
+  for (int r = 0; r < n_ranges; ++r) {
+    const long long off = ranges[2 * r], cnt = ranges[2 * r + 1];
+    if (cnt <= 0 || off < 0 || off > nG || cnt > nG - off) continue;
+    const long long end = off + cnt, a0 = off & ~3LL, nq = (end - a0 + 3) >> 2;
+    for (long long q = gid; q < nq; q += gsz) {
+      const long long base = a0 + 4 * q;
+      if (base >= off && base + 4 <= end) {
+        *reinterpret_cast<float4*>(G + base) = z;
+      } else {
+#pragma unroll
+        for (int e = 0; e < 4; ++e)
+          if (base + e >= off && base + e < end) G[base + e] = 0.f;
+      }
     }
   }
 }
@@ -733,7 +795,18 @@
 extern "C" int mbx_pack_input(const float* img, int64_t pixels, void* out, mbx_stream_t stream) {
   if (!img || !out || pixels <= 0 || !al16(out)) return MBX_ERR_INVALID_ARG;
   MBX_ENTER();
-  hipLaunchKernelGGL(pack_input_kernel, dim3(grid_for(pixels)), dim3(kT), 0, mbx_s(stream), img, (long long)pixels, (us)out);
+  hipLaunchKernelGGL(pack_input_kernel, dim3(grid_for(pixels)), dim3(kT), 0, mbx_s(stream), img, (long long)pixels, (us)out,
+                     (int*)nullptr, 0LL);
+  MBX_LAUNCH_CHECK();
+  return MBX_OK;
+}
+
+extern "C" int mbx_pack_input_clear(const float* img, int64_t pixels, void* out, int32_t* clear, int64_t n_clear,
+                                    mbx_stream_t stream) {
+  if (!img || !out || pixels <= 0 || !al16(out) || n_clear < 0 || (n_clear && !clear)) return MBX_ERR_INVALID_ARG;
+  MBX_ENTER();
+  hipLaunchKernelGGL(pack_input_kernel, dim3(grid_for(pixels)), dim3(kT), 0, mbx_s(stream), img, (long long)pixels, (us)out,
+                     clear, (long long)n_clear);
   MBX_LAUNCH_CHECK();
   return MBX_OK;
 }
@@ -790,6 +863,19 @@
   return MBX_OK;
 }
 
+extern "C" int mbx_head_gather_decode(const mbx_head* heads, int n_heads, int N, int P, const float* priors, float eps_add,
+                                      float* locs, float* logits, float* decoded, float* conf, mbx_stream_t stream) {
+  if (!locs || !logits || !priors || !decoded || !conf || !al16(locs) || !al16(priors) || !al16(decoded)) return MBX_ERR_INVALID_ARG;
+  HeadTable t;
+  const int st = fill_head_table(heads, n_heads, N, P, false, t);
+  if (st != MBX_OK) return st;
+  MBX_ENTER();
+  hipLaunchKernelGGL(head_gather_all_decode_kernel, dim3(grid_for(t.start[t.n])), dim3(kT), 0, mbx_s(stream), t, P,
+                     reinterpret_cast<const float4*>(priors), eps_add, locs, logits, reinterpret_cast<float4*>(decoded), conf);
+  MBX_LAUNCH_CHECK();
+  return MBX_OK;
+}
+
 extern "C" int mbx_head_scatter_all(const float* d_locs, const float* d_logits, const mbx_head* heads, int n_heads, int N,
                                     int P, mbx_stream_t stream) {
   if (!d_locs || !d_logits) return MBX_ERR_INVALID_ARG;
@@ -811,6 +897,21 @@
   hipLaunchKernelGGL(step_begin_kernel, dim3(grid_for((n_grads + n_ws) / 4)), dim3(kT), 0, mbx_s(stream), grads,
                      (long long)n_grads, bn_ws, (long long)n_ws, (long long)ctl_index,
                      reinterpret_cast<unsigned long long*>(timeouts_total), zero_scalar);
+  MBX_LAUNCH_CHECK();
+  return MBX_OK;
+}
+
+extern "C" int mbx_step_begin_ranges(float* grads, int64_t n_grads, int64_t n_head, const int64_t* ranges, int n_ranges,
+                                     int64_t range_elems, float* bn_ws, int64_t n_ws, int64_t ctl_index,
+                                     uint64_t* timeouts_total, float* zero_scalar, mbx_stream_t stream) {
+  if (!grads || n_grads <= 0 || n_head <= 0 || n_head > n_grads || n_head % 4 || n_ws < 0 || n_ws % 4 || (n_ws && !bn_ws) ||
+      !al16(grads) || (bn_ws && !al16(bn_ws)) || n_ranges < 0 || (n_ranges && !ranges) || range_elems < 0 ||
+      (timeouts_total && (ctl_index < 0 || ctl_index >= n_head)))
+    return MBX_ERR_INVALID_ARG;
+  MBX_ENTER();
+  hipLaunchKernelGGL(step_begin_ranges_kernel, dim3(grid_for((n_head + n_ws + range_elems) / 4 + 1)), dim3(kT), 0, mbx_s(stream),
+                     grads, (long long)n_grads, (long long)n_head, reinterpret_cast<const long long*>(ranges), n_ranges, bn_ws,
+                     (long long)n_ws, (long long)ctl_index, reinterpret_cast<unsigned long long*>(timeouts_total), zero_scalar);
   MBX_LAUNCH_CHECK();
   return MBX_OK;
 }
diff --git a/multibox_amd/engine.py b/multibox_amd/engine.py
--- a/multibox_amd/engine.py
+++ b/multibox_amd/engine.py
@@ -163,6 +163,11 @@
         self.B, self.S, self.k, self.mode, self.fine_tune, self.dev = batch, input_size, k, mode, fine_tune, device
         self.bn_decay = bn_decay
         self.tune_registry = []
+        self.decode_into = None
+        self._fwd_cleared = False
+        self._clear_ranges = None
+        self._clear_tables = []
+        self._dw_floats = {}
         self.deterministic = bool(int(os.environ.get("MBX_DETERMINISTIC", "0")))
         self.no_onepass = self.deterministic or bool(int(os.environ.get("MBX_NO_BN_ONEPASS", "0")))
         self.atomic_stats = mode == "train" and not self.deterministic and os.environ.get("MBX_ATOMIC_STATS", "1") != "0"
@@ -749,9 +754,23 @@
                 d = self._desc(op, op.out, epilogue=ops.EPI_STORE_F32)
                 L.append(lambda d=d, op=op: _lib.check(l.mbx_conv(C.byref(d), st()), op.name))
                 if op is self.heads[-1]:
-                    L.append(lambda: _lib.check(l.mbx_head_gather_all(self.head_table, len(self.heads), self.B, self.P,
-                                                                      self.locs.data_ptr(), self.logits.data_ptr(), st()), "head_gather_all"))
+                    def gather():
+                        if self.decode_into is None:
+                            _lib.check(l.mbx_head_gather_all(self.head_table, len(self.heads), self.B, self.P,
+                                                             self.locs.data_ptr(), self.logits.data_ptr(), st()), "head_gather_all")
+                        else:
+                            priors, eps, decoded, conf = self.decode_into
+                            _lib.check(l.mbx_head_gather_decode(self.head_table, len(self.heads), self.B, self.P, priors.data_ptr(),
+                                                                eps, self.locs.data_ptr(), self.logits.data_ptr(),
+                                                                decoded.data_ptr(), conf.data_ptr(), st()), "head_gather_decode")
+                    L.append(gather)
         return L
+
+    def decode_with_gather(self, priors, eps_add, decoded, conf):
+        assert sorted((op.head[2], op.head[2] + op.head[0] * op.head[1]) for op in self.heads)[0][0] == 0 and \
+            sum(op.head[0] * op.head[1] for op in self.heads) == self.P
+        assert priors.shape == (self.P, 4) and decoded.shape == (self.B, self.P, 4) and conf.shape == (self.B, self.P)
+        self.decode_into = (priors, float(eps_add), decoded, conf)
 
     def _bn_forward(self, op):
         l = _lib.lib()
@@ -996,6 +1015,7 @@
             job.dy, job.dy_img_stride, job.ld_dy = dyv.ptr, dyv.img_stride, dyv.ld
             job.scale = float(scale)
             job.dw, job.db = dw.data_ptr(), (None if db is None else db.data_ptr())
+            self._dw_floats[dw.data_ptr()] = dw.numel()
 
             grp = op.group
             if grp is not None and ddesc is not None:
@@ -1029,6 +1049,7 @@
         self.bwd_launches = L
         self.fwd_launches = self._build_forward_launches()
         self._default_groups = None
+        self._clear_ranges = None
 
     def _bn_backward(self, op):
         l = _lib.lib()
@@ -1111,6 +1132,29 @@
     def make_wgrad_groups(self, job_lists):
         return [ops.WgradGroup(jobs, deterministic=self.deterministic, device=self.dev) for jobs in job_lists if jobs]
 
+    def clear_only_for(self, groups):
+        if groups is None:
+            self._clear_ranges = None
+            return None
+        base, stored = self.Wg.data_ptr(), []
+        for g in groups:
+            for ptr, n in g.stored_ranges():
+                lo = (ptr - base) // 4
+                assert (ptr - base) % 4 == 0 and 0 <= lo and lo + n <= self.nW and self._dw_floats.get(ptr) == n, (ptr, n)
+                stored.append((lo, lo + n))
+        ranges, at = [], 0
+        for lo, hi in sorted(stored):
+            assert lo >= at, "two jobs store the same weight gradient"
+            if lo > at:
+                ranges.append((at, lo - at))
+            at = hi
+        if at < self.nW:
+            ranges.append((at, self.nW - at))
+        table = torch.tensor([[self.G_off + lo, n] for lo, n in ranges], dtype=torch.int64).reshape(-1, 2).to(self.dev)
+        self._clear_tables.append(table)
+        self._clear_ranges = (table, ranges, sum(n for _, n in ranges), list(groups))
+        return ranges
+
     def prepare_filters(self):
         if self.mode == "train" and self.filter_entries:
             _lib.check(_lib.lib().mbx_filter_prepare(self.Wb.data_ptr(), self.Wd.data_ptr(), self.filter_table.data_ptr(),
@@ -1135,12 +1179,17 @@
 
     def set_input(self, images_f32):
         assert images_f32.shape == (self.B, self.S, self.S, 3) and images_f32.dtype == torch.float32
-        _lib.check(_lib.lib().mbx_pack_input(images_f32.contiguous().data_ptr(), self.B * self.S * self.S,
-                                             self.images.buf.data_ptr(), torch.cuda.current_stream().cuda_stream), "pack_input")
+        clear = bool(self._i5_used or self.atomic_stats) and isinstance(self._fwd_clear, torch.Tensor)
+        _lib.check(_lib.lib().mbx_pack_input_clear(images_f32.contiguous().data_ptr(), self.B * self.S * self.S,
+                                                   self.images.buf.data_ptr(), self._fwd_clear.data_ptr() if clear else None,
+                                                   self._fwd_clear.numel() if clear else 0,
+                                                   torch.cuda.current_stream().cuda_stream), "pack_input")
+        self._fwd_cleared = clear
 
     def forward(self):
-        if self._i5_used or self.atomic_stats:
+        if (self._i5_used or self.atomic_stats) and not self._fwd_cleared:
             self._fwd_clear.zero_()
+        self._fwd_cleared = False
         for f in self.fwd_launches:
             f()
         return self.locs, self.logits
@@ -1197,6 +1246,13 @@
         return int(self.bn_timeouts_total) + int(float(self.step_ctl[0]))
 
     def zero_grads(self):
+        if self._clear_ranges is not None and not self.fine_tune:
+            table, _, elems, _ = self._clear_ranges
+            _lib.check(_lib.lib().mbx_step_begin_ranges(self.G.data_ptr(), self.G.numel(), self.G_off, table.data_ptr(),
+                                                        table.shape[0], elems, self.bn_ws.data_ptr(), self.bn_ws.numel(),
+                                                        self.nBt, self.bn_timeouts_total.data_ptr(), self.reg_loss.data_ptr(),
+                                                        torch.cuda.current_stream().cuda_stream), "step_begin_ranges")
+            return
         n_clear = self.G_off if self.fine_tune else self.G.numel()
         _lib.check(_lib.lib().mbx_step_begin(self.G.data_ptr(), n_clear, self.bn_ws.data_ptr(), self.bn_ws.numel(),
                                              self.nBt, self.bn_timeouts_total.data_ptr(), self.reg_loss.data_ptr(),
@@ -1216,6 +1272,8 @@
             jobs = [j for j in self.bwd_jobs if j is not None]
             n = max(1, (len(jobs) + 3) // 4)
             self._default_groups = self.make_wgrad_groups([jobs[i:i + n] for i in range(0, len(jobs), n)])
+        assert self._clear_ranges is None or self._clear_ranges[3] == self._default_groups, \
+            "zero_grads() clears for other weight-gradient groups (clear_only_for)"
         for g in self._default_groups:
             g.launch()
 
diff --git a/multibox_amd/loss.py b/multibox_amd/loss.py
--- a/multibox_amd/loss.py
+++ b/multibox_amd/loss.py
@@ -156,6 +156,11 @@
             self.entry, self.entry_args = "mbx_loss_fwd_bwd", ()
             ws_bytes = l.mbx_loss_workspace_bytes(self.B)
         self.ws = torch.empty((ws_bytes,), dtype=torch.uint8, device=device)
+        kind = ("mbx_loss_fwd_bwd", "mbx_loss_fwd_bwd_mined", "mbx_loss_fwd_bwd_focal", "mbx_loss_fwd_bwd_loc").index(self.entry)
+        self.fold_kind = kind
+        self.fold_args = ((self.loc or (0, 0.0)) if kind == 3 else (0, 0.0)) + \
+            ((self.focal or (0.0, 1.0, 1.0)) if kind >= 2 else (0.0, 1.0, 1.0)) + (mining if kind >= 1 else (0, 0, None))
+        self.fold_ws = torch.zeros((l.mbx_loss_folded_workspace_bytes(self.B),), dtype=torch.uint8, device=device)
         self.match_iou_threshold, self.n_extra = match_iou_threshold, None
         if match_iou_threshold is not None:
             if not 0.0 < float(match_iou_threshold) <= 1.0:
@@ -189,11 +194,14 @@
         elif prior_levels is not None:
             raise ValueError("prior_levels is given without atss_topk")
 
-    def forward_backward(self, raw_locs, logits, gt_bboxes, num_gt_bboxes, grad_scale=1.0, conf_is_logit=True):
+    def forward_backward(self, raw_locs, logits, gt_bboxes, num_gt_bboxes, grad_scale=1.0, conf_is_logit=True,
+                         decoded_ready=False):
         l, s = _lib.lib(), _stream()
         B, P, G = self.B, self.P, self.G
         assert raw_locs.shape == (B, P, 4) and logits.numel() == B * P and gt_bboxes.shape == (B, G, 4)
-        if conf_is_logit:
+        if decoded_ready:
+            assert conf_is_logit
+        elif conf_is_logit:
             _lib.check(l.mbx_decode_conf(_f32(raw_locs).data_ptr(), _f32(logits).data_ptr(), self.priors.data_ptr(),
                                          B, P, SMALL_EPSILON, self.decoded.data_ptr(), self.conf.data_ptr(), s),
                        "mbx_decode_conf")
@@ -216,7 +224,8 @@
         common = (self.decoded.data_ptr(), _f32(logits).data_ptr(), int(bool(conf_is_logit)), gt_bboxes.data_ptr(),
                   self.match.data_ptr(), self.alpha, float(grad_scale), B, P, G, self.loss2.data_ptr(), self.d_locs.data_ptr(),
                   self.d_logits.data_ptr())
-        _lib.check(getattr(l, self.entry)(*common, *self.entry_args, self.ws.data_ptr(), self.ws.numel(), s), self.entry)
+        _lib.check(l.mbx_loss_fwd_bwd_folded(self.fold_kind, *common, *self.fold_args, self.fold_ws.data_ptr(),
+                                             self.fold_ws.numel(), s), self.entry + " (folded)")
         return self.loss2, self.d_locs, self.d_logits
 
 
diff --git a/multibox_amd/ops.py b/multibox_amd/ops.py
--- a/multibox_amd/ops.py
+++ b/multibox_amd/ops.py
@@ -395,6 +395,18 @@
         self.host_image = np.frombuffer(host, dtype=np.uint8).copy()
         self.image = torch.from_numpy(self.host_image).to(device)
         self.flops = float(self.info.flops)
+        self.jobs = list(jobs)
+
+    def split_jobs(self):
+        import numpy as np
+        o, n = int(self.info.items_off), int(self.info.n_items)
+        items = self.host_image[o:o + 32 * n].view(np.int32).reshape(n, 8)
+        return sorted(set(int(j) for j in items[items[:, 5] == 0, 0]))
+
+    def stored_ranges(self):
+        split = set(self.split_jobs())
+        return [(int(j.dw), int(j.desc.C_out) * int(j.desc.R) * int(j.desc.S) * int(j.desc.C_in))
+                for i, j in enumerate(self.jobs) if i not in split]
 
     def launch(self, max_workgroups=0):
         _lib.check(_lib.lib().mbx_conv_wgrad_grouped_capped(self.image.data_ptr(), C.byref(self.info), int(max_workgroups),
diff --git a/multibox_amd/trainer.py b/multibox_amd/trainer.py
--- a/multibox_amd/trainer.py
+++ b/multibox_amd/trainer.py
@@ -47,6 +47,8 @@
                                  atss_topk=atss_topk, prior_levels=prior_levels)
         assert self.loss.P == net.P, "priors (%d) do not match the network's predictions (%d)" % (self.loss.P, net.P)
         self.loss.d_locs, self.loss.d_logits = net.d_locs, net.d_logits
+        from .loss import SMALL_EPSILON
+        net.decode_with_gather(self.loss.priors, SMALL_EPSILON, self.loss.decoded, self.loss.conf)
         self.lr0, self.dsteps, self.lr_factor, self.staircase = initial_learning_rate, decay_steps_, learning_rate_decay_factor, staircase
         self.rms_decay, self.momentum, self.eps, self.ema_decay = rmsprop_decay, rmsprop_momentum, rmsprop_epsilon, moving_average_decay
         self.global_step = 0
@@ -327,6 +329,8 @@
         on_gpu = torch.device(net.dev).type == "cuda"
         groups = net.make_wgrad_groups([j for _, _, _, j in segs]) if on_gpu else []
         self.wgrad_groups = groups
+        if on_gpu:
+            net.clear_only_for(groups)
         self._seg_groups, gi = [], 0
         for _, _, _, jobs in segs:
             if jobs and on_gpu:
@@ -349,7 +353,7 @@
             net.zero_grads()
         net.set_input(self.images)
         net.forward()
-        self.loss.forward_backward(net.locs, net.logits, self.gt, self.n_gt)
+        self.loss.forward_backward(net.locs, net.logits, self.gt, self.n_gt, decoded_ready=True)
         if not first:
             net.zero_grads()
 
```

Measured after the change: 4413 images/sec, median of 6. Within noise of the previous version (+0.4%).
